# GeekAlexis/FastMOT

Measured on AMD Instinct MI355X. Metric: end-to-end tracker FPS @1080p/50 dets, higher is better.
Workload: dtype f16

## Files before the change

### fastmot_amd/_lib.py

```python
import ctypes as C
import os
import sys
import weakref
from pathlib import Path

import numpy as np
from types import SimpleNamespace

from .utils.nv12 import NV12Frame
from .utils.jpeg import JPEGFrame, QT_ENTRIES, max_coefficients
from .utils.source import SourceFrame
from .utils.yuv import PlanarFrame, frame_bytes
from .utils.packed import PackedFrame, row_bytes
from .utils.bayer import BayerFrame
from .utils.deep import DeepFrame, deep_frame_bytes
from .utils.devarray import DeviceArrayFrame

LIB_PATH = Path(os.environ.get('FASTMOT_LIB_PATH', Path(__file__).parent / 'libfastmot_hip.so'))

c_int_p = C.POINTER(C.c_int)
_lib = None


class FastMOTHipError(RuntimeError):
# ... 127 lines not shown
    check(load().fm_jpeg_encode_regions_assemble(_ptr(plans), C.c_int(len(plans)), C.c_int(int(quality)), _ptr(lens), _ptr(segs),
                                                 C.c_size_t(segs.size if segs_bytes is None else segs_bytes), _ptr(out), C.c_size_t(cap),
                                                 _ptr(offsets)))
    return [out[int(a):int(b)].tobytes() for a, b in zip(offsets[:-1], offsets[1:])]


def _redact_args(regions):
    regions = np.ascontiguousarray(regions, dtype=REDACT_REGION_DTYPE).reshape(-1)
    return regions, (_ptr(regions) if len(regions) else None, C.c_int(len(regions)))


def redact_check(regions, width, height):
    regions, args = _redact_args(regions)
    return load().fm_redact_check(*args, C.c_int(width), C.c_int(height))


def redact_render_host(frame, regions):
    if not isinstance(frame, np.ndarray) or frame.dtype != np.uint8 or frame.ndim != 3 or frame.shape[2] != 3 or \
            frame.strides[1:] != (3, 1) or frame.strides[0] < 3 * frame.shape[1] or not frame.flags.writeable:
        raise ValueError('frame must be a writeable uint8 HxWx3 array with packed pixels')
    regions, args = _redact_args(regions)
    check(load().fm_redact_render_host(_ptr(frame), C.c_int(frame.shape[1]), C.c_int(frame.shape[0]), C.c_size_t(frame.strides[0]), *args))
    return frame


def device_count():
    n = load().fm_device_count()
    if n < 0:
        raise FastMOTHipError(load().fm_last_error().decode())
    return n


def device_pci_bus_id(device):
    buf = C.create_string_buffer(64)
    check(load().fm_device_pci_bus_id(C.c_int(device), buf, C.c_int(64)))
    return buf.value.decode().lower()


class HipContext:

    def __init__(self, device=0):
        self._dev_pending = []
        self.lib = load()
        self._ctx = C.c_void_p()
        check(self.lib.fm_ctx_create(C.c_int(device), C.byref(self._ctx)))
        self.device = device
        self.feat_dim = 512

    def close(self):
        if getattr(self, '_ctx', None) is not None and self._ctx:
            self.lib.fm_ctx_destroy(self._ctx)
            self._ctx = C.c_void_p()
        for frame, _ in self._dev_pending:
            frame._pending = [(ref, t) for ref, t in frame._pending if ref() is not self]
        self._dev_pending = []

    def __del__(self):
        if sys.is_finalizing():
            return
        try:
            self.close()
        except Exception:
            pass

    @property
    def handle(self):
        return self._ctx

    def synchronize(self):
        check(self.lib.fm_ctx_synchronize(self._ctx))

    def set_option(self, key, value):
        check(self.lib.fm_ctx_set_option(self._ctx, key.encode(), C.c_int(int(value))))

    def get_option(self, key):
        v = C.c_int(0)
        check(self.lib.fm_ctx_get_option(self._ctx, key.encode(), C.byref(v)))
        return v.value

    def front_info(self):
        k, b, n = C.c_int(0), C.c_longlong(0), C.c_longlong(0)
        check(self.lib.fm_net_front_info(self._ctx, C.byref(k), C.byref(b), C.byref(n)))
        return k.value, b.value, n.value

    def trace_start(self, cap=20000):
        t0 = C.c_int64(0)
        check(self.lib.fm_trace_start(self._ctx, C.c_int(cap), C.byref(t0)))
        self._trace_cap = cap
        return t0.value

    def trace_read(self):
        cap = self._trace_cap
        tags = np.zeros(cap, np.int32)
        ms = np.zeros(cap, np.float32)
        n = C.c_int(0)
        check(self.lib.fm_trace_read(self._ctx, C.c_int(cap), _ptr(tags), _ptr(ms), C.byref(n)))
        return tags[:n.value], ms[:n.value]

    def bind_thread(self):
        check(self.lib.fm_ctx_bind_thread(self._ctx))

    def device_info(self):
        buf = C.create_string_buffer(256)
        check(self.lib.fm_device_info(self._ctx, buf, 256))
        parts = buf.value.decode().split(':')
        return {'name': parts[0], 'arch': ':'.join(parts[1:-3]), 'cus': int(parts[-3]),
                'clock_mhz': int(parts[-2]), 'hbm_bytes': int(parts[-1])}

    def kf_configure(self, dt, std_factor_acc, std_offset_acc, std_factor_det, std_factor_klt,
                     min_std_det, min_std_klt, init_pos_weight, init_vel_weight, vel_coupling,
                     vel_half_life):
        p = KFParams(dt, std_factor_acc, std_offset_acc, (C.c_double * 2)(*std_factor_det),
                     (C.c_double * 2)(*std_factor_klt), (C.c_double * 2)(*min_std_det),
                     (C.c_double * 2)(*min_std_klt), init_pos_weight, init_vel_weight, vel_coupling,
                     vel_half_life)
        check(self.lib.fm_kf_configure(self._ctx, C.byref(p)))

    def set_frame_rect(self, tlbr):
        a = _as(tlbr, np.float64, (4,))
        check(self.lib.fm_set_frame_rect(self._ctx, _ptr(a)))

    def trk_create(self, slots, det_tlbr):
        s = _as(slots, np.int32)
        b = _as(det_tlbr, np.float64, (-1, 4))
        assert len(s) == len(b)
        check(self.lib.fm_trk_create(self._ctx, C.c_int(len(s)), _ptr(s), _ptr(b)))

    def trk_step(self, slots, H, klt_tlbr, has_klt, mult):
        s = _as(slots, np.int32)
        n = len(s)
        Hm = _as(H, np.float64, (9,))
        k = _as(klt_tlbr, np.float64, (-1, 4)) if n else np.zeros((0, 4))
        hk = _as(has_klt, np.uint8)
        mu = _as(mult, np.float64)
        assert len(k) == n and len(hk) == n and len(mu) == n
        tlbr = np.empty((n, 4), np.float64)
        lost = np.empty(n, np.uint8)
        check(self.lib.fm_trk_step(self._ctx, C.c_int(n), _ptr(s), _ptr(Hm), _ptr(k), _ptr(hk),
                                   _ptr(mu), _ptr(tlbr), _ptr(lost)))
        return tlbr, lost.astype(bool)

    def trk_step_ops(self, ops, slots, H, klt_tlbr, has_klt, mult):
        s = _as(slots, np.int32)
        n = len(s)
        Hm = _as(H, np.float64, (9,))
        k = _as(klt_tlbr, np.float64, (-1, 4)) if n else np.zeros((0, 4))
        hk = _as(has_klt, np.uint8)
        mu = _as(mult, np.float64)
        tlbr = np.empty((n, 4), np.float64)
        lost = np.empty(n, np.uint8)
        check(self.lib.fm_trk_step_ops(self._ctx, C.c_int(ops), C.c_int(n), _ptr(s), _ptr(Hm), _ptr(k),
                                       _ptr(hk), _ptr(mu), _ptr(tlbr), _ptr(lost)))
        return tlbr, lost.astype(bool)

    def trk_update_det(self, slots, det_tlbr):
        s = _as(slots, np.int32)
        n = len(s)
        b = _as(det_tlbr, np.float64, (-1, 4)) if n else np.zeros((0, 4))
        assert len(b) == n
        tlbr = np.empty((n, 4), np.float64)
        lost = np.empty(n, np.uint8)
        check(self.lib.fm_trk_update_det(self._ctx, C.c_int(n), _ptr(s), _ptr(b), _ptr(tlbr), _ptr(lost)))
        return tlbr, lost.astype(bool)

    def trk_get_state(self, slots):
        s = _as(slots, np.int32)
# ... 931 lines not shown
```

### fastmot_amd/build.py

```python
import subprocess
import sys
from pathlib import Path

PKG = Path(__file__).resolve().parent
CSRC = PKG / 'csrc'
OUT = PKG / 'libfastmot_hip.so'
HIPCC = '/opt/rocm/bin/hipcc'
import os
FLAGS = ['--offload-arch=gfx950', '-O3', '-std=c++17', '-fPIC', '-shared', '-ffp-contract=off',
         '-Wno-unused-result'] + os.environ.get('FASTMOT_EXTRA_HIPCC_FLAGS', '').split()


FILE_FLAGS = {'flow.hip': ['-fno-slp-vectorize'], 'diag.hip': ['-fno-slp-vectorize'], 'reidhead_gem.hip': ['-fno-slp-vectorize']}


def sources():
    return sorted(CSRC.glob('*.hip'))


FLAGS_STAMP = PKG / 'build' / 'flags.txt'


def needs_build():
    if not OUT.exists():
        return True
    if not FLAGS_STAMP.exists() or FLAGS_STAMP.read_text() != ' '.join(FLAGS):
        return True
    t = OUT.stat().st_mtime
    deps = list(CSRC.glob('*')) + [PKG.parent / 'include' / 'fastmot_hip.h', Path(__file__)]
    return any(p.stat().st_mtime > t for p in deps)


def build(force=False, verbose=True):
    if not force and not needs_build():
        return OUT
    if FLAGS_STAMP.exists() and FLAGS_STAMP.read_text() != ' '.join(FLAGS):
        force = True
    objs = []
    procs = []
    bdir = PKG / 'build'
    bdir.mkdir(exist_ok=True)
    for src in sources():
        obj = bdir / (src.stem + '.o')
        objs.append(obj)
        if not force and obj.exists() and obj.stat().st_mtime > max(
                src.stat().st_mtime, *(h.stat().st_mtime for h in CSRC.glob('*.h')),
                (PKG.parent / 'include' / 'fastmot_hip.h').stat().st_mtime):
            continue
        cmd = [HIPCC] + [f for f in FLAGS if f != '-shared'] + FILE_FLAGS.get(src.name, []) + ['-c', str(src), '-o', str(obj)]
        procs.append((src, subprocess.Popen(cmd, stdout=subprocess.PIPE, stderr=subprocess.STDOUT)))
    for src, p in procs:
        out, _ = p.communicate()
        if p.returncode != 0:
            raise RuntimeError(f'hipcc failed on {src}:\n{out.decode()}')
        if verbose and out.strip():
            print(out.decode())
    cmd = [HIPCC, '--offload-arch=gfx950', '-shared', '-fPIC', '-o', str(OUT)] + [str(o) for o in objs]
    res = subprocess.run(cmd, stdout=subprocess.PIPE, stderr=subprocess.STDOUT)
    if res.returncode != 0:
        raise RuntimeError(f'link failed:\n{res.stdout.decode()}')
    FLAGS_STAMP.write_text(' '.join(FLAGS))
    if verbose:
        print(f'built {OUT}')
    return OUT


if __name__ == '__main__':
    build(force='--force' in sys.argv)
```

### fastmot_amd/csrc/common.h

```cpp
#pragma once
#include <hip/hip_runtime.h>
#include <atomic>
#include <cstdarg>
#include <cstdint>
#include <cstdio>
#include <cstring>
#include <string>
#include <vector>
#include "../../include/fastmot_hip.h"
#ifdef FM_DIAG
#include "../../include/fastmot_hip_diag.h"
#endif

#define FM_ERR_HIP (-1)
#define FM_ERR_ARG (-2)
#define FM_ERR_STATE (-3)

void fm_set_error(const char* fmt, ...);

#define FM_HIP(call)                                                                        \
    do {                                                                                    \
        hipError_t e_ = (call);                                                             \
        if (e_ != hipSuccess) {                                                             \
            fm_set_error("%s:%d %s -> %s", __FILE__, __LINE__, #call, hipGetErrorString(e_)); \
            return FM_ERR_HIP;                                                              \
        }                                                                                   \
    } while (0)

#define FM_CHECK_ARG(cond)                                                     \
    do {                                                                       \
        if (!(cond)) {                                                         \
            fm_set_error("%s:%d bad argument: %s", __FILE__, __LINE__, #cond); \
            return FM_ERR_ARG;                                                 \
        }                                                                      \
    } while (0)

bool fm_lap_host(const double* cost, int nr, int nc, long rs, long cs, int32_t* col4row_out);
int fm_greedy_host(const double* cost, int nr, int nc, double max_cost, int32_t* m_rows, int32_t* m_cols);
#define FM_ZERO_COPY_TRACKS (ctx->opt_zero_copy_tracks)

struct DevBuf {
    void* d = nullptr;
    void* h = nullptr;
    size_t cap = 0;
    bool pinned_mirror = true;
    int reserve(size_t bytes) {
        if (bytes <= cap) return 0;
        size_t ncap = cap ? cap : 4096;
        while (ncap < bytes) ncap *= 2;
        if (d) (void)hipFree(d);
        if (h) (void)hipHostFree(h);
        d = h = nullptr;
        cap = 0;
        FM_HIP(hipMalloc(&d, ncap));
        if (pinned_mirror) FM_HIP(hipHostMalloc(&h, ncap, hipHostMallocDefault));
        cap = ncap;
        return 0;
    }
    void release() {
        if (d) (void)hipFree(d);
        if (h) (void)hipHostFree(h);
        d = h = nullptr;
        cap = 0;
    }
    template <typename T> T* dev() { return reinterpret_cast<T*>(d); }
    template <typename T> T* host() { return reinterpret_cast<T*>(h); }
};

struct KFConst {
    double F_pos_self;
    double F_pos_other;
    double F_vel;
    double q_pp, q_pv, q_vv;
    double std_factor_acc, std_offset_acc;
    double fac_det[2], fac_klt[2], min_det[2], min_klt[2];
    double init_pos_weight, init_vel_weight;
};

struct NetState;
struct DetState;
struct ExtState;
struct FlowState;
struct EncState;
struct OvlState;
struct YuvState;
struct SsdState;
struct GalleryState;
constexpr int FM_GALLERY_CHANNELS = 2;

struct fm_ctx {
    int device = 0;
    int opt_zero_copy_tracks = 2048;
    int opt_host_lap_elems = 262144;
    int opt_use_graphs = 1;
    int opt_fused_input = 1;
    int opt_net_timing = 0;
    int opt_nms_general = 0;
    int opt_det_front_ahead = 1;
    int opt_det_front_layers = -1;
    int opt_det_front_stream = 0;
    bool det_flush_deferred = false;
    int opt_lk_variant = 0;
    void* predict_worker = nullptr;
    hipStream_t s_main = nullptr;
    hipStream_t s_det = nullptr;
    hipStream_t s_up = nullptr;
    hipStream_t s_ext = nullptr;
    hipStream_t s_ext_x[FM_MAX_EXTRA_EXTRACTORS] = {};
    hipEvent_t ev_ext_in = nullptr, ev_ext_x_done[FM_MAX_EXTRA_EXTRACTORS] = {};
    hipStream_t s_flow = nullptr;
    hipStream_t s_flow2 = nullptr;
    hipEvent_t ev_pyr = nullptr;
    bool pyr_pending = false;
    hipEvent_t ev_prep = nullptr, ev_bg = nullptr;
    hipEvent_t ev_feat = nullptr;
    hipEvent_t ev_ext_net = nullptr;
    hipEvent_t ev_ext_done = nullptr;
    hipEvent_t ev_pair = nullptr;
    bool ext_net_recorded = false;
    size_t as_in_bytes = 0;
    bool as_in_device = true;
    bool as_mirror = false;

    int slot_cap = 0;
    double* mean = nullptr;
    double* cov = nullptr;
    int feat_dim = 512;
    float* feat_sum = nullptr;
    float* feat_avg = nullptr;
    int32_t* feat_cnt = nullptr;
    KFConst kf{};
    bool kf_set = false;
    double frame_rect[4] = {0, 0, 0, 0};

    float* emb = nullptr;
    float* emb_host = nullptr;
    int emb_cap = 0;
    int emb_n = 0;

    int as_nT = 0, as_nD = 0, as_metric = 0;
    size_t as_off[6] = {0, 0, 0, 0, 0, 0};
    DevBuf as_in;
    DevBuf as_pair;
    DevBuf as_stage_in;
    DevBuf as_cost;
    DevBuf as_work;
    DevBuf as_out;
    DevBuf io0, io1;
    DevBuf occ_in, occ_out;
    DevBuf feat_in;

    int frame_w = 0, frame_h = 0, ring_size = 0;
    uint8_t* frame_cur = nullptr;
    uint8_t* frame_own = nullptr;
    uint8_t* frame_own2 = nullptr;
    uint8_t* frame_next = nullptr;
    uint8_t* frame_pinned2 = nullptr;
    hipEvent_t ev_next_upload = nullptr;
    uint8_t* frame_ahead[FM_MAX_DET_BATCH + 1] = {};
    uint8_t* frame_up[FM_MAX_DET_BATCH + 1] = {};
    uint8_t* frame_up_pinned[FM_MAX_DET_BATCH + 1] = {};
    hipEvent_t ev_up[FM_MAX_DET_BATCH + 1] = {};
    uint8_t* frame_ring = nullptr;
    uint8_t* frame_pinned = nullptr;

    DetState* det = nullptr;
    SsdState* ssd = nullptr;
    ExtState* ext = nullptr;
    NetState* det_net = nullptr;
    NetState* ext_net = nullptr;
    NetState* ext_net_x[FM_MAX_EXTRA_EXTRACTORS] = {};
    FlowState* flow = nullptr;
    EncState* enc = nullptr;
    OvlState* ovl = nullptr;
    YuvState* yuv = nullptr;
    GalleryState* gallery[2] = {nullptr, nullptr};

    std::vector<hipEvent_t> trace_ev;
// ... 123 lines not shown
```

### fastmot_amd/csrc/convd.hip

```cpp
#include "net.h"
#include <atomic>
#include <cstdlib>

int launch_convd(const ConvParams& p, hipStream_t s);

namespace {

int g_convd_cfg = 0;

#ifdef FM_CONVD_TIMING
__device__ long long g_convd_stamps[2][264];
int g_convd_abl = 0;
#define CONVD_STAMP(i) if (stamp_slot >= 0 && (i) < 264) reinterpret_cast<long long*>(smem + stamp_off)[(i)] = __builtin_readcyclecounter();
#define CONVD_ABL(bit) (abl & (bit))
#define CONVD_EXTRA_PARAM , const int abl, const int stamp_off
#define CONVD_EXTRA_ARG , g_convd_abl, (int)lds
#define CONVD_EXTRA_LDS 4096
#else
#define CONVD_STAMP(i)
#define CONVD_ABL(bit) false
#define CONVD_EXTRA_PARAM
#define CONVD_EXTRA_ARG
#define CONVD_EXTRA_LDS 0
#endif
// ... 195 lines not shown
#pragma unroll
                        for (int pi = 0; pi < MP; ++pi)
                            acc[mi][pi] = __builtin_amdgcn_mfma_f32_32x32x16_f16(af[mi], bf[pi], acc[mi][pi], 0, 0, 0);
                }
            }
            c_stage = c_stage + 1 == nslots ? 0 : c_stage + 1;
        }
        CONVD_STAMP(11 + 4 * it)
    }
    CONVD_STAMP(3)

    if constexpr (KG > 1) {
        __syncthreads();
        float4* part = reinterpret_cast<float4*>(smem + BN * LDO * 4);
        if (mfma_wave && g > 0) {
#pragma unroll
            for (int mi = 0; mi < MC; ++mi)
#pragma unroll
                for (int pi = 0; pi < MP; ++pi)
#pragma unroll
                    for (int q = 0; q < 4; ++q)
                        part[(((g - 1) * MC * MP + mi * MP + pi) * 4 + q) * 256 + w * 64 + lane] =
                            make_float4(acc[mi][pi][4 * q + 0], acc[mi][pi][4 * q + 1], acc[mi][pi][4 * q + 2], acc[mi][pi][4 * q + 3]);
        }
        __syncthreads();
        if (mfma_wave && g == 0) {
            for (int gg = 1; gg < KG; ++gg)
#pragma unroll
                for (int mi = 0; mi < MC; ++mi)
#pragma unroll
                    for (int pi = 0; pi < MP; ++pi)
#pragma unroll
                        for (int q = 0; q < 4; ++q) {
                            const float4 t4 = part[(((gg - 1) * MC * MP + mi * MP + pi) * 4 + q) * 256 + w * 64 + lane];
                            acc[mi][pi][4 * q + 0] += t4.x; acc[mi][pi][4 * q + 1] += t4.y;
                            acc[mi][pi][4 * q + 2] += t4.z; acc[mi][pi][4 * q + 3] += t4.w;
                        }
        }
    }
    CONVD_STAMP(4)
    float* so = reinterpret_cast<float*>(smem);
    if constexpr (KG == 1) __syncthreads();
    if (mfma_wave && g == 0) {
#pragma unroll
        for (int pi = 0; pi < MP; ++pi)
#pragma unroll
            for (int mi = 0; mi < MC; ++mi)
#pragma unroll
                for (int q = 0; q < 4; ++q)
                    *reinterpret_cast<float4*>(&so[((wp * MP + pi) * 32 + frow) * LDO + (wc * MC + mi) * 32 + 8 * q + 4 * fh]) =
                        make_float4(acc[mi][pi][4 * q + 0], acc[mi][pi][4 * q + 1], acc[mi][pi][4 * q + 2], acc[mi][pi][4 * q + 3]);
    }
    __syncthreads();
    constexpr int CH = BM / 8;
    constexpr int ROWS = T / CH;
    const int och = tid % CH, orow = tid / CH;
    const int co = c0 + och * 8;
    if (co < p.cout_store && !CONVD_ABL(4)) {
        const int hw_out = p.Ho * p.Wo;
        const float inv_hw = 1.f / (float)hw_out, inv_wo = 1.f / (float)p.Wo;
        float bias8[8];
        *reinterpret_cast<float4*>(&bias8[0]) = *reinterpret_cast<const float4*>(p.bias + co);
        *reinterpret_cast<float4*>(&bias8[4]) = *reinterpret_cast<const float4*>(p.bias + co + 4);
        constexpr int NPASS = (BN + ROWS - 1) / ROWS;
        float v[NPASS][8], r[NPASS][8];
#pragma unroll
        for (int ps = 0; ps < NPASS; ++ps) {
            const int row = min(orow + ps * ROWS, BN - 1);
            *reinterpret_cast<float4*>(&v[ps][0]) = *reinterpret_cast<const float4*>(&so[row * LDO + och * 8]);
            *reinterpret_cast<float4*>(&v[ps][4]) = *reinterpret_cast<const float4*>(&so[row * LDO + och * 8 + 4]);
        }
        if (p.res_mode != RES_NONE) {
#pragma unroll
            for (int ps = 0; ps < NPASS; ++ps) {
                const int pix = min(p0 + orow + ps * ROWS, p.P - 1);
                unpack8(*reinterpret_cast<const uint4*>(p.res + (size_t)pix * p.res_cs + p.res_coff + co), r[ps]);
            }
        }
#pragma unroll
        for (int ps = 0; ps < NPASS; ++ps) {
            const int row = orow + ps * ROWS;
            const int pix = p0 + row;
            if (row >= BN || pix >= p.P) continue;
#pragma unroll
            for (int e = 0; e < 8; ++e) {
                v[ps][e] += bias8[e];
                if (p.res_mode == RES_BEFORE_ACT) v[ps][e] += r[ps][e];
            }
            apply_act_n<8>(v[ps], p.act);
            if (p.res_mode == RES_AFTER_ACT) {
#pragma unroll
                for (int e = 0; e < 8; ++e) v[ps][e] += r[ps][e];
            }
            if (p.out32) {
                float* dst = p.out32 + (size_t)pix * p.out_cs + p.out_coff + co;
                *reinterpret_cast<float4*>(dst) = make_float4(v[ps][0], v[ps][1], v[ps][2], v[ps][3]);
                *reinterpret_cast<float4*>(dst + 4) = make_float4(v[ps][4], v[ps][5], v[ps][6], v[ps][7]);
            } else {
                const uint4 o = pack8(v[ps]);
                if (p.up == 2) {
                    const int nn = idiv_small(pix, hw_out, inv_hw), rem = pix - nn * hw_out;
                    const int ry = idiv_small(rem, p.Wo, inv_wo), rx = rem - ry * p.Wo;
                    const size_t o00 = ((size_t)nn * 2 * p.Ho + 2 * ry) * (2 * p.Wo) + 2 * rx;
                    f16* dst = p.out + o00 * p.out_cs + p.out_coff + co;
                    *reinterpret_cast<uint4*>(dst) = o;
                    *reinterpret_cast<uint4*>(dst + p.out_cs) = o;
                    *reinterpret_cast<uint4*>(dst + (size_t)2 * p.Wo * p.out_cs) = o;
                    *reinterpret_cast<uint4*>(dst + (size_t)(2 * p.Wo + 1) * p.out_cs) = o;
                } else {
                    *reinterpret_cast<uint4*>(p.out + (size_t)pix * p.out_cs + p.out_coff + co) = o;
                }
            }
        }
    }
    CONVD_STAMP(5)
#ifdef FM_CONVD_TIMING
    if (stamp_slot >= 0) {
        long long* st = reinterpret_cast<long long*>(smem + stamp_off);
        st[263] = __builtin_amdgcn_s_memrealtime();
        st[6] = per;
        st[7] = BM * 1000000 + BN * 1000 + KG * 100 + SPB * 10 + ns;
        for (int i = 0; i < 264; ++i) g_convd_stamps[stamp_slot][i] = st[i];
    }
#endif
#endif
}

constexpr int LDS_MAX = 160 * 1024;

struct Cfg {
    int bm, bn, kg, ns, role, spb;
};

template <int WC, int WP, int MC, int MP, int KG, int TAPS, int ROLE, int SPB>
int launch_inst(const ConvParams& p, int ns, hipStream_t s) {
    constexpr int BM = WC * MC * 32, BN = WP * MP * 32, SS = (BM + BN) * 128 * SPB;
    const int cout_pad = (p.Cout + 31) & ~31;
    const int nk = p.Kpad >> 6, per = ((nk + KG - 1) / KG + SPB - 1) / SPB;
    const int nslots = ns < per ? ns : (per < 1 ? 1 : per);
    ConvParams q = p;
    q.grid_p = (p.P + BN - 1) / BN;
    q.grid_c = (cout_pad + BM - 1) / BM;
    q.grid_z = 1;
    q.weight_major = (size_t)cout_pad * p.Kpad > (size_t)p.N * p.H * p.W * p.Cin ? 1 : 0;
    const size_t ring = (size_t)KG * nslots * SS;
    const size_t epi = (size_t)BN * (BM + 4) * 4 + (size_t)(KG - 1) * BM * BN * 4;
    const size_t lds = ring > epi ? ring : epi;
    FM_CHECK_ARG(lds + CONVD_EXTRA_LDS <= (size_t)LDS_MAX);
    static std::atomic<unsigned long long> configured{0};
    int dev = 0;
    FM_HIP(hipGetDevice(&dev));
    if (dev >= 64 || !(configured.load(std::memory_order_relaxed) >> dev & 1)) {
        FM_HIP(hipFuncSetAttribute(reinterpret_cast<const void*>(convd_kernel<WC, WP, MC, MP, KG, TAPS, ROLE, SPB>),
                                   hipFuncAttributeMaxDynamicSharedMemorySize, LDS_MAX));
        if (dev < 64) configured.fetch_or(1ull << dev, std::memory_order_relaxed);
    }
    const int total = q.grid_p * q.grid_c;
    hipLaunchKernelGGL((convd_kernel<WC, WP, MC, MP, KG, TAPS, ROLE, SPB>), dim3(((total + 7) / 8) * 8), dim3(256 * KG * (1 + ROLE)),
                       lds + CONVD_EXTRA_LDS, s, q, ns, nslots CONVD_EXTRA_ARG);
    FM_HIP(hipGetLastError());
    return 0;
}

template <int MC, int MP, int KG, int ROLE, int SPB>
int launch_taps(const ConvParams& p, int ns, hipStream_t s) {
    if (p.KH == 1) return launch_inst<2, 2, MC, MP, KG, 0, ROLE, SPB>(p, ns, s);
    return launch_inst<2, 2, MC, MP, KG, 3, ROLE, SPB>(p, ns, s);
}

template <int MC, int MP, int SPB>
int launch_role(const ConvParams& p, const Cfg& c, hipStream_t s) {
    if constexpr (MC * MP == 1 && SPB == 1) {
        if (c.kg == 4) return launch_taps<MC, MP, 4, 0, 1>(p, c.ns, s);
    }
    if (c.kg >= 2) return c.role ? launch_taps<MC, MP, 2, 1, SPB>(p, c.ns, s) : launch_taps<MC, MP, 2, 0, SPB>(p, c.ns, s);
    return c.role ? launch_taps<MC, MP, 1, 1, SPB>(p, c.ns, s) : launch_taps<MC, MP, 1, 0, SPB>(p, c.ns, s);
// ... 88 lines not shown
```

### fastmot_amd/csrc/ctx.hip

```cpp
#include <algorithm>
#include "common.h"
void convd_set_cfg(int code);
#include <sched.h>
#include <cstring>
#include <cstdlib>
#include <cmath>

static thread_local char g_err[1024] = "";

void fm_set_error(const char* fmt, ...) {
    va_list ap;
    va_start(ap, fmt);
    vsnprintf(g_err, sizeof(g_err), fmt, ap);
    va_end(ap);
}

extern "C" const char* fm_last_error(void) { return g_err; }

extern "C" int fm_ctx_set_option(fm_ctx* ctx, const char* key, int value) {
    FM_CHECK_ARG(ctx && key && (value >= 0 || (value == -1 && !strcmp(key, "det_front_layers"))));
    if (!strcmp(key, "zero_copy_tracks")) ctx->opt_zero_copy_tracks = value;
    else if (!strcmp(key, "host_lap_elems")) ctx->opt_host_lap_elems = value;
    else if (!strcmp(key, "use_graphs")) ctx->opt_use_graphs = value;
    else if (!strcmp(key, "convd_cfg")) convd_set_cfg(value);
    else if (!strcmp(key, "nms_path")) {
        ctx->opt_nms_general = value != 0;
    }
    else if (!strcmp(key, "fused_input")) ctx->opt_fused_input = value != 0;
    else if (!strcmp(key, "net_timing")) ctx->opt_net_timing = value;
    else if (!strcmp(key, "det_front_ahead") || !strcmp(key, "det_front_stream")) {
        FM_CHECK_ARG(value <= (key[10] == 'a' ? 2 : 1));
        (key[10] == 'a' ? ctx->opt_det_front_ahead : ctx->opt_det_front_stream) = value;
    }
    else if (!strcmp(key, "det_front_layers")) ctx->opt_det_front_layers = value;
    else if (!strcmp(key, "lk_variant")) {
#ifndef FM_DIAG
        if (value != 0) {
            fm_set_error("option 'lk_variant' needs a diagnostic build of the library (-DFM_DIAG)");
            return FM_ERR_ARG;
        }
#endif
        ctx->opt_lk_variant = value;
    }
    else {
        fm_set_error("unknown option '%s'", key);
        return FM_ERR_ARG;
    }
    return 0;
}

extern "C" int fm_ctx_get_option(fm_ctx* ctx, const char* key, int* value) {
    FM_CHECK_ARG(ctx && key && value);
    if (!strcmp(key, "det_front_ahead")) *value = ctx->opt_det_front_ahead;
    else if (!strcmp(key, "det_front_layers")) *value = ctx->opt_det_front_layers;
    else if (!strcmp(key, "det_front_stream")) *value = ctx->opt_det_front_stream;
    else {
        fm_set_error("option '%s' cannot be read", key);
        return FM_ERR_ARG;
    }
    return 0;
}

extern "C" int fm_trace_start(fm_ctx* ctx, int cap, int64_t* host_ns) {
    FM_CHECK_ARG(ctx && cap > 0 && host_ns && !ctx->trace_on.load() && ctx->trace_ev.empty());
    FM_HIP(hipDeviceSynchronize());
    std::vector<hipEvent_t> evs(cap);
    for (auto& e : evs) FM_HIP(hipEventCreate(&e));
    if (!ctx->trace_base) FM_HIP(hipEventCreate(&ctx->trace_base));
    FM_HIP(hipEventRecord(ctx->trace_base, ctx->s_main));
    FM_HIP(hipEventSynchronize(ctx->trace_base));
    timespec ts;
    clock_gettime(CLOCK_MONOTONIC, &ts);
    *host_ns = (int64_t)ts.tv_sec * 1000000000ll + ts.tv_nsec;
    ctx->trace_tag.assign(cap, 0);
    ctx->trace_n = 0;
    ctx->trace_ev = std::move(evs);
    ctx->trace_on.store(true, std::memory_order_release);
    return 0;
}

extern "C" int fm_trace_read(fm_ctx* ctx, int cap, int32_t* tags, float* ms, int* n) {
    FM_CHECK_ARG(ctx && tags && ms && n);
    ctx->trace_on.store(false, std::memory_order_seq_cst);
    while (ctx->trace_busy.load(std::memory_order_seq_cst) > 0) sched_yield();
    FM_HIP(hipDeviceSynchronize());
    std::vector<hipEvent_t> evs = std::move(ctx->trace_ev);
    ctx->trace_ev.clear();
    int k = ctx->trace_n.load();
    if (k > (int)evs.size()) k = (int)evs.size();
    if (k > cap) k = cap;
    for (int i = 0; i < k; ++i) {
        tags[i] = ctx->trace_tag[i];
        FM_HIP(hipEventElapsedTime(&ms[i], ctx->trace_base, evs[i]));
    }
    *n = k;
    for (auto& e : evs) (void)hipEventDestroy(e);
    return 0;
}

extern "C" int fm_ctx_bind_thread(fm_ctx* ctx) {
    FM_CHECK_ARG(ctx);
    FM_HIP(hipSetDevice(ctx->device));
    return 0;
}

extern "C" int fm_device_pci_bus_id(int device, char* buf, int buflen) {
    FM_CHECK_ARG(buf && buflen >= 16);
    FM_HIP(hipDeviceGetPCIBusId(buf, buflen, device));
    return 0;
}

extern "C" int fm_device_count(void) {
    int n = 0;
    FM_HIP(hipGetDeviceCount(&n));
    return n;
}

void fm_net_free(NetState* n);
void fm_det_free(DetState* d);
void fm_ext_free(ExtState* e);
void fm_flow_free(FlowState* f);

extern "C" int fm_ctx_create(int device, fm_ctx** out) {
    FM_CHECK_ARG(out != nullptr);
    int n = 0;
    FM_HIP(hipGetDeviceCount(&n));
    if (device < 0 || device >= n) {
        fm_set_error("device %d out of range (%d visible)", device, n);
        return FM_ERR_ARG;
    }
    FM_HIP(hipSetDevice(device));
    fm_ctx* ctx = new fm_ctx();
    ctx->device = device;
    if (const char* e = getenv("FASTMOT_ZERO_COPY")) ctx->opt_zero_copy_tracks = atoi(e);
    if (const char* e = getenv("FASTMOT_HOST_LAP")) ctx->opt_host_lap_elems = atoi(e);
    if (const char* e = getenv("FASTMOT_GRAPHS")) ctx->opt_use_graphs = atoi(e);
    if (const char* e = getenv("FASTMOT_FUSED_INPUT")) ctx->opt_fused_input = atoi(e) != 0;
    if (const char* e = getenv("FASTMOT_FRONT_AHEAD")) ctx->opt_det_front_ahead = std::min(std::max(atoi(e), 0), 2);
    if (const char* e = getenv("FASTMOT_FRONT_STREAM")) ctx->opt_det_front_stream = atoi(e) == 1;
    int prio_lo = 0, prio_hi = 0;
    FM_HIP(hipDeviceGetStreamPriorityRange(&prio_lo, &prio_hi));
    const int prio_det = prio_lo, prio_ext = prio_hi;
    FM_HIP(hipStreamCreateWithPriority(&ctx->s_main, hipStreamNonBlocking, prio_hi));
    FM_HIP(hipStreamCreateWithPriority(&ctx->s_det, hipStreamNonBlocking, prio_det));
    FM_HIP(hipStreamCreateWithPriority(&ctx->s_up, hipStreamNonBlocking, prio_lo));
    FM_HIP(hipStreamCreateWithPriority(&ctx->s_ext, hipStreamNonBlocking, prio_ext));
    FM_HIP(hipEventCreateWithFlags(&ctx->ev_ext_in, hipEventDisableTiming));
    for (int i = 0; i < FM_MAX_EXTRA_EXTRACTORS; ++i) {
        FM_HIP(hipStreamCreateWithPriority(&ctx->s_ext_x[i], hipStreamNonBlocking, prio_hi));
        FM_HIP(hipEventCreateWithFlags(&ctx->ev_ext_x_done[i], hipEventDisableTiming));
    }
    FM_HIP(hipStreamCreateWithPriority(&ctx->s_flow, hipStreamNonBlocking, prio_hi));
    FM_HIP(hipStreamCreateWithPriority(&ctx->s_flow2, hipStreamNonBlocking, prio_hi));
    FM_HIP(hipEventCreateWithFlags(&ctx->ev_pyr, hipEventDisableTiming));
    FM_HIP(hipEventCreateWithFlags(&ctx->ev_prep, hipEventDisableTiming));
    FM_HIP(hipEventCreateWithFlags(&ctx->ev_bg, hipEventDisableTiming));
    FM_HIP(hipEventCreateWithFlags(&ctx->ev_feat, hipEventDisableTiming));
    FM_HIP(hipEventCreateWithFlags(&ctx->ev_ext_net, hipEventDisableTiming));
    FM_HIP(hipEventCreateWithFlags(&ctx->ev_pair, hipEventDisableTiming));
    FM_HIP(hipEventCreateWithFlags(&ctx->ev_ext_done, hipEventDisableTiming));
    int rc = fm_ensure_slots(ctx, 1024);
    if (rc) return rc;
    *out = ctx;
    return 0;
}

extern "C" int fm_ctx_destroy(fm_ctx* ctx) {
    if (!ctx) return 0;
    (void)hipSetDevice(ctx->device);
    fm_predict_worker_free(ctx);
    fm_gallery_free(ctx);
    (void)hipDeviceSynchronize();
    if (ctx->det) fm_det_free(ctx->det);
    fm_ssd_free(ctx);
    if (ctx->ext) fm_ext_free(ctx->ext);
    for (void* p : {(void*)ctx->frame_own, (void*)ctx->frame_own2, (void*)ctx->frame_ring})
        if (p) (void)hipFree(p);
    if (ctx->frame_pinned) (void)hipHostFree(ctx->frame_pinned);
    if (ctx->frame_pinned2) (void)hipHostFree(ctx->frame_pinned2);
    for (int k = 2; k <= FM_MAX_DET_BATCH; ++k) {
        if (ctx->frame_up[k]) (void)hipFree(ctx->frame_up[k]);
        if (ctx->frame_up_pinned[k]) (void)hipHostFree(ctx->frame_up_pinned[k]);
        if (ctx->ev_up[k]) (void)hipEventDestroy(ctx->ev_up[k]);
    }
    for (hipEvent_t e : ctx->ev_jpeg)
        if (e) (void)hipEventDestroy(e);
    fm_frame_dev_free(ctx);
    fm_frame_staging_free(ctx);
    fm_overlay_free(ctx);
    fm_yuv_free(ctx);
    fm_jpegenc_free(ctx);
    if (ctx->det_net) fm_net_free(ctx->det_net);
    if (ctx->ext_net) fm_net_free(ctx->ext_net);
    for (NetState* x : ctx->ext_net_x)
        if (x) fm_net_free(x);
    if (ctx->flow) fm_flow_free(ctx->flow);
    for (void* p : {(void*)ctx->mean, (void*)ctx->cov, (void*)ctx->feat_sum, (void*)ctx->feat_avg,
                    (void*)ctx->feat_cnt, (void*)ctx->emb})
        if (p) (void)hipFree(p);
    if (ctx->emb_host) (void)hipHostFree(ctx->emb_host);
    for (DevBuf* b : {&ctx->as_in, &ctx->as_pair, &ctx->as_stage_in, &ctx->as_cost, &ctx->as_work,
                      &ctx->as_out, &ctx->io0, &ctx->io1, &ctx->feat_in, &ctx->occ_in, &ctx->occ_out})
        b->release();
    for (hipStream_t s : {ctx->s_main, ctx->s_det, ctx->s_up, ctx->s_ext, ctx->s_flow, ctx->s_flow2})
        if (s) (void)hipStreamDestroy(s);
    for (hipEvent_t e : {ctx->ev_feat, ctx->ev_ext_in, ctx->ev_pyr, ctx->ev_prep, ctx->ev_bg, ctx->ev_ext_net, ctx->ev_pair, ctx->ev_ext_done})
        if (e) (void)hipEventDestroy(e);
    for (int i = 0; i < FM_MAX_EXTRA_EXTRACTORS; ++i) {
        if (ctx->s_ext_x[i]) (void)hipStreamDestroy(ctx->s_ext_x[i]);
        if (ctx->ev_ext_x_done[i]) (void)hipEventDestroy(ctx->ev_ext_x_done[i]);
    }
    delete ctx;
    return 0;
}

extern "C" int fm_ctx_synchronize(fm_ctx* ctx) {
    FM_CHECK_ARG(ctx);
    FM_HIP(hipStreamSynchronize(ctx->s_main));
    FM_HIP(hipStreamSynchronize(ctx->s_det));
    FM_HIP(hipStreamSynchronize(ctx->s_up));
// ... 345 lines not shown
```

### fastmot_amd/csrc/detect.hip

```cpp
#include "pixel_source.h"
#include <cmath>
#include <string>
#include <vector>

struct DetState {
    fm_yolo_cfg cfg{};
    bool configured = false;
    int cap = 8192;
    static constexpr int NSLOT_UNTILED = FM_MAX_DET_BATCH + 2;
    static constexpr int NSLOT = 3 * FM_MAX_DET_BATCH;
    int nslot = NSLOT_UNTILED;
    int n_tiles = 0;
    int tile_x[FM_MAX_DET_BATCH] = {}, tile_y[FM_MAX_DET_BATCH] = {};
    int region_w = 0, region_h = 0;
    double tile_offset[FM_MAX_DET_BATCH][2] = {};
    double merge_thresh = 0.6;
    std::vector<fm_det48> tile_stage;
    std::vector<fm_det48> tile_dets;
    std::vector<int32_t> tile_ids;
    int tile_count[FM_MAX_DET_BATCH] = {};
    int tile_sum[2] = {};
    float* cand[NSLOT] = {};
    float* sorted[NSLOT] = {};
    int32_t* counters[NSLOT] = {};
// ... 606 lines not shown
}

static int detect_ahead(fm_ctx* ctx, int n) {
    FM_CHECK_ARG(ctx && ctx->det_net && n >= 1 && n <= FM_MAX_DET_BATCH);
    if (n > ctx->det_net->max_batch) {
        fm_set_error("detector look-ahead of %d frames > the detector network's max_batch %d", n, ctx->det_net->max_batch);
        return FM_ERR_ARG;
    }
    const uint8_t* frames[FM_MAX_DET_BATCH];
    hipEvent_t uploads[FM_MAX_DET_BATCH];
    for (int k = 1; k <= n; ++k) {
        frames[k - 1] = fm_ahead_frame(ctx, k);
        if (!frames[k - 1]) {
            fm_set_error("look-ahead slot %d holds no frame (fm_frame_upload_ahead / fm_frame_ring_select_ahead)", k);
            return FM_ERR_ARG;
        }
        uploads[k - 1] = frames[k - 1] == fm_ahead_buf(ctx, k) ? fm_ahead_event(ctx, k) : nullptr;
    }
    return detect_pass(ctx, frames, uploads, n, true);
}

static int detect_pass(fm_ctx* ctx, const uint8_t* const* frames, const hipEvent_t* uploads, int n, bool look_ahead) {
    FM_CHECK_ARG(ctx && ctx->det && ctx->det->configured && ctx->det_net);
    DetState* d = ctx->det;
    NetState* net = ctx->det_net;
    const fm_yolo_cfg& c = d->cfg;
    const bool tiled = d->n_tiles > 1;
    const int n_frames = n;
    if (tiled) {
        FM_CHECK_ARG(n_frames == 1);
        n = d->n_tiles;
        if (n > net->max_batch) {
            fm_set_error("%d tiles > the detector network's max_batch %d", n, net->max_batch);
            return FM_ERR_ARG;
        }
    }
    FM_CHECK_ARG(n >= 1 && n <= FM_MAX_DET_BATCH && n <= net->max_batch);
    hipStream_t s = ctx->s_det;
    int rc = 0;
    const bool fused = ctx->opt_fused_input && fm_net_stem_fusable(net, c.input_tensor);
    int K = 0;
    if (ctx->det_flush_deferred && !(look_ahead && fused && n == 1 && !tiled)) {
        ctx->det_flush_deferred = false;
        if ((rc = flush_post(ctx, d))) return rc;
    }
    if (look_ahead && fused && n == 1 && !tiled && ctx->opt_det_front_ahead && ctx->opt_det_front_layers) {
        bool busy = ctx->opt_det_front_ahead == 2;
        if (!busy && d->pending > 0 && hipEventQuery(d->ev_dec[(d->wr + d->nslot - 1) % d->nslot]) != hipSuccess) {
            (void)hipGetLastError();
            busy = true;
        }
        if (busy && (rc = fm_net_front_prepare(ctx, net, ctx->opt_det_front_layers, &K))) return rc;
    }
    if (ctx->det_flush_deferred && !K) {
        ctx->det_flush_deferred = false;
        if ((rc = flush_post(ctx, d))) return rc;
    }
    const bool timing = ctx->opt_net_timing > 0 && d->n_passes++ % ctx->opt_net_timing == 0;
    for (int i = 0; i < n; ++i) {
        d->timed[(d->wr + i) % d->nslot] = timing && i == 0;
        d->timed_front[(d->wr + i) % d->nslot] = timing && i == 0 && K > 0;
    }
    struct Restore {
        NetState* net;
        ~Restore() { net->first = net->last = 0; fm_net_select(net, nullptr, net->set); }
    } restore{net};
    fm_trace_mark(ctx, s, 10);
    if (K > 0) {
        hipStream_t se = ctx->opt_det_front_stream == 1 ? ctx->s_ext : ctx->s_up;
        const int set = net->set ^ 1;
        if (net->front_stream && net->front_stream != se) FM_HIP(hipStreamSynchronize(net->front_stream));
        net->front_stream = se;
        ++net->front_passes;
        if (uploads[0] && se != ctx->s_ext) FM_HIP(hipStreamWaitEvent(se, uploads[0], 0));
        if ((rc = acquire_slots(ctx, d, se, 1))) return rc;
        if (d->set_slot[set] >= 0 && hipEventQuery(d->ev_dec[d->set_slot[set]]) != hipSuccess) {
            (void)hipGetLastError();
            FM_HIP(hipStreamWaitEvent(se, d->ev_dec[d->set_slot[set]], 0));
        }
        const StemSrc src = det_source(ctx, d, frames, n);
        fm_net_select(net, se, set);
        if (timing) FM_HIP(hipEventRecord(d->evf0[d->wr], se));
        fm_trace_mark(ctx, se, 11);
        if ((rc = fm_net_run_stem_from(ctx, net, src, n))) return rc;
        fm_trace_mark(ctx, se, 15);
        if (K > 1) {
            net->first = 1;
            net->last = K;
            if ((rc = fm_net_run_internal(ctx, FM_NET_DETECTOR, n))) return rc;
        }
        if (timing) FM_HIP(hipEventRecord(d->evf1[d->wr], se));
        fm_trace_mark(ctx, se, 16);
        FM_HIP(hipEventRecord(d->ev_front[set], se));
        if (ctx->det_flush_deferred) {
            ctx->det_flush_deferred = false;
            if ((rc = flush_post(ctx, d))) return rc;
        }
        fm_net_select(net, nullptr, set);
        FM_HIP(hipStreamWaitEvent(s, d->ev_front[set], 0));
        fm_trace_mark(ctx, s, 14);
        if (timing) FM_HIP(hipEventRecord(d->ev0[d->wr], s));
        net->first = K;
        net->last = 0;
        if ((rc = fm_net_run_internal(ctx, FM_NET_DETECTOR, n))) return rc;
        net->first = 0;
    } else {
        for (int i = 0; i < n_frames; ++i)
            if (uploads[i]) FM_HIP(hipStreamWaitEvent(s, uploads[i], 0));
        if ((rc = acquire_slots(ctx, d, s, n))) return rc;
        fm_trace_mark(ctx, s, 14);
        const StemSrc src = det_source(ctx, d, frames, n);
        if (fused) {
            if (timing) FM_HIP(hipEventRecord(d->ev0[d->wr], s));
            fm_trace_mark(ctx, s, 11);
            if ((rc = fm_net_run_stem_from(ctx, net, src, n))) return rc;
            fm_trace_mark(ctx, s, 15);
            net->first = 1;
            rc = fm_net_run_internal(ctx, FM_NET_DETECTOR, n);
            net->first = 0;
            if (rc) return rc;
        } else {
            if ((rc = enqueue_preprocess(ctx, d, net, src, n))) return rc;
            if (timing) FM_HIP(hipEventRecord(d->ev0[d->wr], s));
            fm_trace_mark(ctx, s, 11);
            if ((rc = fm_net_run_internal(ctx, FM_NET_DETECTOR, n))) return rc;
        }
    }
    d->set_slot[net->set] = d->wr;
    if (timing) FM_HIP(hipEventRecord(d->ev1[d->wr], s));
    fm_trace_mark(ctx, s, 12);
    FilterArgs fa = filter_args(d, d->wr);
    HeadSet hs{};
    for (int i = 0; i < n; ++i) {
        const int slot = (d->wr + i) % d->nslot;
        hs.cand[i] = d->cand[slot];
        hs.counters[i] = d->counters[slot];
    }
    for (int i = 0; i < FM_MAX_DET_BATCH; ++i) {
        hs.off_x[i] = tiled && i < n ? d->tile_offset[i][0] : c.offset[0];
        hs.off_y[i] = tiled && i < n ? d->tile_offset[i][1] : c.offset[1];
    }
    int base = 0, blocks = 0;
    for (int i = 0; i < FM_MAX_HEADS + 1; ++i) hs.first_block[i] = 0x7fffffff;
    for (int i = 0; i < c.n_heads; ++i) {
        FM_CHECK_ARG(c.head_tensor[i] >= 0 && c.head_tensor[i] < (int)net->tensors.size());
        const fm_tensor& t = net->tensors[c.head_tensor[i]];
        FM_CHECK_ARG(t.f32 && t.h == c.grid_h[i] && t.w == c.grid_w[i] && c.n_anchors[i] <= FM_MAX_ANCHORS);
        HeadArgs& h = hs.h[i];
        h.data = (const float*)net->bufs[c.head_tensor[i]];
        h.cs = t.c; h.gw = c.grid_w[i]; h.gh = c.grid_h[i]; h.na = c.n_anchors[i];
        h.base_index = base;
        memcpy(h.anchors, c.anchors[i], sizeof(float) * 2 * FM_MAX_ANCHORS);
        h.scale_xy = c.scale_xy[i];
        const int cnt = h.gw * h.gh * h.na;
        hs.first_block[i] = blocks;
        blocks += (cnt + 255) / 256;
        base += cnt;
    }
    if (blocks) hipLaunchKernelGGL(decode_kernel, dim3(blocks, n), dim3(256), 0, s, hs, fa, c.in_w, c.in_h, c.new_coords);
    FM_HIP(hipGetLastError());
    fm_trace_mark(ctx, s, 13);
    return enqueue_post(ctx, d, s, n);
}

extern "C" int fm_detect_sync(fm_ctx* ctx, fm_det48* out, int cap, int* n) {
    FM_CHECK_ARG(ctx && ctx->det && ctx->det->configured && out && n);
    if (ctx->det->n_tiles > 1) return collect_tiles(ctx, ctx->det, ctx->s_det, out, cap, n);
    return collect(ctx, ctx->det, ctx->s_det, out, cap, n);
}

extern "C" int fm_filter_dets(fm_ctx* ctx, const float* rows, int n, fm_det48* out, int cap, int* n_out) {
    FM_CHECK_ARG(ctx && ctx->det && ctx->det->configured && n >= 0 && out && n_out);
    FM_CHECK_ARG(n < (1 << FM_SORT_INDEX_BITS));
    DetState* d = ctx->det;
    hipStream_t s = ctx->s_det;
    FM_HIP(hipStreamSynchronize(s));
    FM_HIP(hipStreamSynchronize(ctx->s_up));
    if (int rc_n = fm_net_sync(ctx->det_net)) return rc_n;
    d->set_slot[0] = d->set_slot[1] = -1;
    d->post_pending = -1;
    d->post_pending_n = 0;
    d->rd = d->wr;
    d->pending = 0;
    if (n > d->rows_cap) {
        if (d->rows_in) FM_HIP(hipFree(d->rows_in));
        d->rows_in = nullptr;
        FM_HIP(hipMalloc(&d->rows_in, sizeof(float) * 7 * (size_t)n));
        d->rows_cap = n;
    }
    if (n) FM_HIP(hipMemcpyAsync(d->rows_in, rows, sizeof(float) * 7 * (size_t)n, hipMemcpyHostToDevice, s));
    FM_HIP(hipMemsetAsync(d->counters[d->wr], 0, sizeof(int32_t) * 4, s));
    if (n) hipLaunchKernelGGL(rows_filter_kernel, dim3((n + 255) / 256), dim3(256), 0, s, d->rows_in, n, filter_args(d, d->wr));
    int rc = enqueue_post(ctx, d, s);
    if (rc) return rc;
    return collect(ctx, d, s, out, cap, n_out);
}

extern "C" int fm_detect_last_counts(fm_ctx* ctx, int* n_candidates, int* n_detections) {
    FM_CHECK_ARG(ctx && ctx->det && n_candidates && n_detections);
    const DetState* d = ctx->det;
// ... 56 lines not shown
```

### fastmot_amd/csrc/extract.hip

```cpp
#include "pixel_source.h"
#include <cmath>

struct ExtState {
    int input_tensor = -1, in_w = 0, in_h = 0;
    double* boxes = nullptr;
    double* boxes_host = nullptr;
    int cap = 0;
    DevBuf emb_out;
    int exported_n = -1;
    bool mirror_export = false;
};

void fm_ext_invalidate_export(fm_ctx* ctx) {
    if (ctx->ext) ctx->ext->exported_n = -1;
}

void fm_ext_free(ExtState* e) {
    if (!e) return;
    e->emb_out.release();
    if (e->boxes) (void)hipFree(e->boxes);
    if (e->boxes_host) (void)hipHostFree(e->boxes_host);
    delete e;
}

namespace {

__global__ __launch_bounds__(256) void export_kernel(const float4* __restrict__ src, float4* __restrict__ dst, int n4) {
    for (int i = blockIdx.x * 256 + threadIdx.x; i < n4; i += gridDim.x * 256) dst[i] = src[i];
}

__global__ void crop_resize_kernel(const uint8_t* __restrict__ frame, int fw, int fh,
                                   const double* __restrict__ boxes, int n, f16* __restrict__ out,
                                   int ow, int oh, int cs) {
    const int x = blockIdx.x * blockDim.x + threadIdx.x;
    const int y = blockIdx.y, b = blockIdx.z;
    if (x >= ow) return;
    f16x8 o;
    crop_input_pixel(frame, fw, fh, boxes + (size_t)b * 4, x, y, ow, oh, o);
    *reinterpret_cast<f16x8*>(out + (((size_t)b * oh + y) * ow + x) * cs) = o;
}

}

extern "C" int fm_extract_configure(fm_ctx* ctx, int input_tensor, int in_w, int in_h) {
    FM_CHECK_ARG(ctx && ctx->ext_net && input_tensor >= 0 && input_tensor < (int)ctx->ext_net->tensors.size());
    const fm_tensor& t = ctx->ext_net->tensors[input_tensor];
    FM_CHECK_ARG(t.h == in_h && t.w == in_w && !t.f32);
    if (!ctx->ext) ctx->ext = new ExtState();
    ctx->ext->input_tensor = input_tensor;
    ctx->ext->in_w = in_w;
    ctx->ext->in_h = in_h;
    return 0;
}

int fm_emb_reserve(fm_ctx* ctx, int n);
bool fm_net_writes_mirror(const NetState* net);

static int export_embeddings(fm_ctx* ctx, ExtState* e, int n, hipStream_t s) {
    const size_t bytes = sizeof(float) * (size_t)n * ctx->feat_dim;
    e->exported_n = -1;
    if (ctx->emb_host && fm_net_writes_mirror(ctx->ext_net)) {
        e->exported_n = n;
        e->mirror_export = true;
        FM_HIP(hipEventRecord(ctx->ev_ext_done, s));
        return 0;
    }
    e->mirror_export = false;
    if (bytes > e->emb_out.cap) {
        FM_HIP(hipStreamSynchronize(s));
        int rc = e->emb_out.reserve(bytes);
        if (rc) return rc;
    }
    const int n4 = (int)(bytes / 16);
    hipLaunchKernelGGL(export_kernel, dim3((n4 + 255) / 256 < 64 ? (n4 + 255) / 256 : 64), dim3(256), 0, s,
                       (const float4*)ctx->emb, (float4*)e->emb_out.h, n4);
    FM_HIP(hipGetLastError());
    e->exported_n = n;
    FM_HIP(hipEventRecord(ctx->ev_ext_done, s));
    return 0;
}

static int front_end(fm_ctx* ctx, ExtState* e, NetState* ni, hipStream_t si, int off, int b, int cs) {
    ni->first = 0;
    if (ctx->opt_fused_input && fm_net_stem_fusable(ni, e->input_tensor)) {
        StemSrc src{};
        src.kind = 2; src.frame[0] = ctx->frame_cur; src.fw = ctx->frame_w; src.fh = ctx->frame_h;
        src.boxes = e->boxes_host + (size_t)off * 4;
        int rc = fm_net_run_stem_from(ctx, ni, src, b);
        if (rc) return rc;
        ni->first = 1;
        return 0;
    }
    hipLaunchKernelGGL(crop_resize_kernel, dim3((e->in_w + 127) / 128, e->in_h, b), dim3(128), 0, si,
                       ctx->frame_cur, ctx->frame_w, ctx->frame_h, e->boxes + (size_t)off * 4, b,
                       (f16*)ni->bufs[e->input_tensor], e->in_w, e->in_h, cs);
    FM_HIP(hipGetLastError());
    return 0;
}

extern "C" int fm_extract_async(fm_ctx* ctx, int n, const double* tlbr) {
    FM_CHECK_ARG(ctx && ctx->ext && ctx->ext_net && n >= 0 && ctx->frame_cur);
    ctx->emb_n = 0;
    ctx->ext_net_recorded = false;
    int rc_exp = 0;
    if (ctx->ext) ctx->ext->exported_n = -1;
    if (n == 0) return 0;
    FM_CHECK_ARG(tlbr);
    ExtState* e = ctx->ext;
    NetState* net = ctx->ext_net;
    hipStream_t s = ctx->s_ext;
    if (n > e->cap) {
        FM_HIP(hipStreamSynchronize(s));
        if (e->boxes) FM_HIP(hipFree(e->boxes));
        if (e->boxes_host) FM_HIP(hipHostFree(e->boxes_host));
        e->boxes = e->boxes_host = nullptr;
        int cap = e->cap ? e->cap : 64;
        while (cap < n) cap *= 2;
        FM_HIP(hipMalloc(&e->boxes, sizeof(double) * 4 * cap));
        FM_HIP(hipHostMalloc(&e->boxes_host, sizeof(double) * 4 * cap, hipHostMallocDefault));
        e->cap = cap;
    }
    if (hipEventQuery(ctx->ev_feat) != hipSuccess) {
        (void)hipGetLastError();
        FM_HIP(hipStreamWaitEvent(s, ctx->ev_feat, 0));
    }
    if (n > ctx->emb_cap) {
        FM_HIP(hipStreamSynchronize(ctx->s_main));
        FM_HIP(hipStreamSynchronize(s));
        int rc = fm_emb_reserve(ctx, n);
        if (rc) return rc;
    }
    FM_HIP(hipStreamSynchronize(s));
    memcpy(e->boxes_host, tlbr, sizeof(double) * 4 * n);
    const bool zero_copy_boxes = ctx->opt_fused_input && fm_net_stem_fusable(net, e->input_tensor);
    if (!zero_copy_boxes)
        FM_HIP(hipMemcpyAsync(e->boxes, e->boxes_host, sizeof(double) * 4 * n, hipMemcpyHostToDevice, s));
    fm_trace_mark(ctx, s, 32);
    const fm_tensor& t = net->tensors[e->input_tensor];
    int parts = 1;
    while (parts <= FM_MAX_EXTRA_EXTRACTORS && ctx->ext_net_x[parts - 1]) ++parts;
    while (parts > 1 && n < 4 * parts) --parts;
    if (parts > 1 && (n + parts - 1) / parts <= net->max_batch) {
        FM_HIP(hipEventRecord(ctx->ev_ext_in, s));
        int off = 0;
        for (int i = 0; i < parts; ++i) {
            const int b = n / parts + (i < n % parts ? 1 : 0);
            NetState* ni = i == 0 ? net : ctx->ext_net_x[i - 1];
            hipStream_t si = i == 0 ? s : ctx->s_ext_x[i - 1];
            FM_CHECK_ARG(b <= ni->max_batch);
            if (i) FM_HIP(hipStreamWaitEvent(si, ctx->ev_ext_in, 0));
            int rc = front_end(ctx, e, ni, si, off, b, t.c);
            if (rc) return rc;
            ni->emb_offset = off;
            rc = fm_net_run_internal(ctx, i == 0 ? FM_NET_EXTRACTOR : FM_NET_EXTRACTOR_B + i - 1, b);
            ni->emb_offset = 0;
            ni->first = 0;
            if (rc) return rc;
            if (i) {
                FM_HIP(hipEventRecord(ctx->ev_ext_x_done[i - 1], si));
                FM_HIP(hipStreamWaitEvent(s, ctx->ev_ext_x_done[i - 1], 0));
            }
            off += b;
        }
        FM_HIP(hipEventRecord(ctx->ev_ext_net, s));
        ctx->ext_net_recorded = true;
        if ((rc_exp = export_embeddings(ctx, e, n, s))) return rc_exp;
        fm_trace_mark(ctx, s, 33);
        ctx->emb_n = n;
        return 0;
    }
    for (int off = 0; off < n; off += net->max_batch) {
        const int b = n - off < net->max_batch ? n - off : net->max_batch;
        int rc = front_end(ctx, e, net, s, off, b, t.c);
// ... 61 lines not shown
```

### fastmot_amd/csrc/net.h

```cpp
#pragma once
#include "common.h"
#include <hip/hip_fp16.h>

typedef _Float16 f16;
typedef f16 f16x8 __attribute__((ext_vector_type(8)));
typedef f16 f16x4 __attribute__((ext_vector_type(4)));
typedef float f32x16 __attribute__((ext_vector_type(16)));
typedef float f32x4 __attribute__((ext_vector_type(4)));

enum { ACT_LINEAR = 0, ACT_LEAKY = 1, ACT_MISH = 2, ACT_RELU = 3, ACT_LOGISTIC = 4, ACT_SWISH = 5, ACT_RELU6 = 6 };
enum { RES_NONE = 0, RES_AFTER_ACT = 1, RES_BEFORE_ACT = 2 };

struct ConvParams {
    const f16* in;  int in_cs, in_coff;
    const f16* w;
    const float* bias;
    f16* out;       int out_cs, out_coff;
    float* out32;
    const f16* res; int res_cs, res_coff;
    int N, H, W, Cin, Ho, Wo, Cout, KH, KW, stride, pad;
    int K, Kpad, P;
    int cout_store;
    int act, res_mode;
    int grid_p, grid_c, grid_z, weight_major;
    int pad_dx;
    int up;
    int batch_inv;
};

int launch_conv(const ConvParams& p, float* ws, size_t ws_floats, hipStream_t s);

struct NetState {
    int which = 0, max_batch = 0;
    std::vector<fm_tensor> tensors;
    std::vector<void*> bufs;
    std::vector<fm_layer> layers;
    char* weights = nullptr;
    size_t weight_bytes = 0;
    float* gates = nullptr;
    int n_gates = 0, gate_c = 0;
    hipStream_t stream = nullptr;
    char* arena = nullptr;
    float* ws = nullptr;
    size_t ws_floats = 0;
    struct GraphKey {
        long batch_emb;
        int first, last, set;
        bool operator==(const GraphKey& o) const { return batch_emb == o.batch_emb && first == o.first && last == o.last && set == o.set; }
    };
    std::vector<std::pair<GraphKey, hipGraphExec_t>> graphs;
    bool use_graphs = true;
    int emb_offset = 0;
    int batch_offset = 0;
    int first = 0;
    int last = 0;
    int front_k = 0;
    int front_req = 0;
    int set = 0;
    std::vector<void*> bufs_b;
    std::vector<char> in_front;
    std::vector<void*> front_owned;
    float* ws_b = nullptr;
    size_t front_bytes = 0;
    hipStream_t home = nullptr;
    hipStream_t front_stream = nullptr;
    long front_passes = 0;
};

int fm_net_front_prepare(fm_ctx* ctx, NetState* net, int request, int* k);
void fm_net_select(NetState* net, hipStream_t s, int set);
int fm_net_sync(NetState* net);

NetState* fm_net_get(fm_ctx* ctx, int which);
int fm_net_run_internal(fm_ctx* ctx, int which, int batch);

__device__ __forceinline__ void unpack8(const uint4& v, float* f) {
    const f16x8 h = *reinterpret_cast<const f16x8*>(&v);
#pragma unroll
    for (int e = 0; e < 8; ++e) f[e] = (float)h[e];
}
__device__ __forceinline__ uint4 pack8(const float* f) {
    f16x8 h;
#pragma unroll
    for (int e = 0; e < 8; ++e) h[e] = (f16)f[e];
    return *reinterpret_cast<const uint4*>(&h);
}

__device__ __forceinline__ int idiv_small(int i, int d, float inv) {
    (void)d;
    return (int)(((float)i + 0.5f) * inv);
}

template <int HI>
__device__ __forceinline__ float fma_mix_h(uint32_t packed, float k, float acc) {
    float d;
    if constexpr (HI) asm("v_fma_mix_f32 %0, %1, %2, %3 op_sel:[1,0,0] op_sel_hi:[1,0,0]" : "=v"(d) : "v"(packed), "v"(k), "v"(acc));
    else asm("v_fma_mix_f32 %0, %1, %2, %3 op_sel:[0,0,0] op_sel_hi:[1,0,0]" : "=v"(d) : "v"(packed), "v"(k), "v"(acc));
    return d;
}
template <int HI>
__device__ __forceinline__ float fma_mix_hh(uint32_t packed, uint32_t kpacked, float acc) {
    float d;
    if constexpr (HI) asm("v_fma_mix_f32 %0, %1, %2, %3 op_sel:[1,1,0] op_sel_hi:[1,1,0]" : "=v"(d) : "v"(packed), "v"(kpacked), "v"(acc));
    else asm("v_fma_mix_f32 %0, %1, %2, %3 op_sel:[0,0,0] op_sel_hi:[1,1,0]" : "=v"(d) : "v"(packed), "v"(kpacked), "v"(acc));
    return d;
}
template <int N>
__device__ __forceinline__ void fma_mix_nh(const uint32_t* raw, const uint32_t* k, float* acc) {
#pragma unroll
    for (int e = 0; e < N; e += 2) {
        acc[e] = fma_mix_hh<0>(raw[e >> 1], k[e >> 1], acc[e]);
        acc[e + 1] = fma_mix_hh<1>(raw[e >> 1], k[e >> 1], acc[e + 1]);
    }
}
template <int N>
__device__ __forceinline__ void fma_mix_n(const uint32_t* raw, const float* k, float* acc) {
#pragma unroll
    for (int e = 0; e < N; e += 2) {
        acc[e] = fma_mix_h<0>(raw[e >> 1], k[e], acc[e]);
        acc[e + 1] = fma_mix_h<1>(raw[e >> 1], k[e + 1], acc[e + 1]);
    }
}

__device__ __forceinline__ void store_out(const ConvParams& p, long pix, int co, f16x4 o) {
    if (p.up == 2) {
        const int hw = p.Ho * p.Wo, rem = (int)(pix % hw);
        const size_t o00 = ((size_t)(pix / hw) * 2 * p.Ho + 2 * (rem / p.Wo)) * (2 * p.Wo) + 2 * (rem % p.Wo);
        f16* dst = p.out + o00 * p.out_cs + p.out_coff + co;
        *reinterpret_cast<f16x4*>(dst) = o;
        *reinterpret_cast<f16x4*>(dst + p.out_cs) = o;
        *reinterpret_cast<f16x4*>(dst + (size_t)2 * p.Wo * p.out_cs) = o;
        *reinterpret_cast<f16x4*>(dst + (size_t)(2 * p.Wo + 1) * p.out_cs) = o;
    } else {
        *reinterpret_cast<f16x4*>(p.out + (size_t)pix * p.out_cs + p.out_coff + co) = o;
    }
}

__device__ __forceinline__ float act_rcp(float x) { return __builtin_amdgcn_rcpf(x); }
__device__ __forceinline__ float act_leaky(float x) { return x > 0.f ? x : 0.1f * x; }
__device__ __forceinline__ float act_relu(float x) { return x > 0.f ? x : 0.f; }
__device__ __forceinline__ float act_relu6(float x) { return fminf(fmaxf(x, 0.f), 6.f); }
__device__ __forceinline__ float act_mish(float x) {
    const float n = __expf(x);
    const float t = n * (n + 2.f);
    return x > 20.f ? x : x * (t * act_rcp(t + 2.f));
}
__device__ __forceinline__ float act_logistic(float x) { return act_rcp(1.f + __expf(-x)); }
__device__ __forceinline__ float act_swish(float x) { return x * act_rcp(1.f + __expf(-x)); }

__device__ __forceinline__ float apply_act(float x, int act) {
    switch (act) {
        case ACT_LEAKY: return act_leaky(x);
        case ACT_MISH: return act_mish(x);
        case ACT_RELU: return act_relu(x);
        case ACT_LOGISTIC: return act_logistic(x);
        case ACT_SWISH: return act_swish(x);
        case ACT_RELU6: return act_relu6(x);
        default: return x;
    }
}

template <int N>
__device__ __forceinline__ void apply_act_n(float* v, int act) {
    switch (act) {
        case ACT_LEAKY:
#pragma unroll
            for (int e = 0; e < N; ++e) v[e] = act_leaky(v[e]);
            break;
        case ACT_MISH:
#pragma unroll
            for (int e = 0; e < N; ++e) v[e] = act_mish(v[e]);
            break;
        case ACT_RELU:
#pragma unroll
            for (int e = 0; e < N; ++e) v[e] = act_relu(v[e]);
            break;
        case ACT_LOGISTIC:
#pragma unroll
            for (int e = 0; e < N; ++e) v[e] = act_logistic(v[e]);
            break;
        case ACT_SWISH:
#pragma unroll
            for (int e = 0; e < N; ++e) v[e] = act_swish(v[e]);
            break;
        case ACT_RELU6:
#pragma unroll
            for (int e = 0; e < N; ++e) v[e] = act_relu6(v[e]);
            break;
        default: break;
    }
}
```

### fastmot_amd/csrc/net.hip

```cpp
#include "pixel_source.h"
#include <algorithm>
#include <memory>

int launch_dwconv3(const f16* in, int in_cs, int in_coff, f16* out, int out_cs, int out_coff, const f16* w,
                   const float* bias, int N, int H, int W, int C, int act, hipStream_t s);
int launch_dwconv(const f16* in, int in_cs, int in_coff, f16* out, int out_cs, int out_coff, const f16* w,
                  const float* bias, int N, int H, int W, int Ho, int Wo, int C, int stride, int act, hipStream_t s);
bool sepconv_supported(int cin, int cout, int stride);
int launch_sepconv(const f16* in, int in_cs, int in_coff, f16* out, int out_cs, int out_coff, const f16* wdw,
                   const float* bdw, const f16* wpw, const float* bpw, int N, int H, int W, int Ho, int Wo, int cin,
                   int cout, int stride, int act1, int act2, long p_choice, hipStream_t s);
int launch_liteconv(int G, const f16* const* in, const int* in_cs, const int* in_coff, f16* out, int out_cs,
                    int out_coff, const f16* wpw, int kpad, const f16* wdw, const float* bias, int N, int H,
                    int W, int C, int act, float* gap_out, hipStream_t s);
void liteconv_tiling(int C, int W, int H, int* th, int* tw, int* tiles_x, int* tiles_y);
int launch_litechain(const f16* in, int in_cs, int in_coff, f16* out, int out_cs, int out_coff, const f16* wpw,
                     int kpad, const f16* wdw, const float* bias, int N, int H, int W, int C, int act,
                     float* const* gap, hipStream_t s);
int launch_gated_sum(int nstreams, const f16* const* in, const int* in_cs, const int* in_coff, int N, int HW,
                     int C, int hid, const f16* w1, const float* b1, const f16* w2, const float* b2, f16* out,
                     int out_cs, int out_coff, const float* const* part, int tiles, hipStream_t s);
constexpr int GATE_SLOT_TILES = 32;
int launch_pair11(const f16* xa, int xa_cs, int xa_coff, const f16* xc, int xc_cs, int xc_coff, f16* out, int out_cs,
                  int out_coff, const f16* w1, const float* b1, const f16* w2, const float* b2, long P, int cout, int act1,
                  int act2, hipStream_t s, long p_choice);
bool pair11_supported(int cin, int mid, int extra, int cout);
int launch_ostail(const f16* in, int in_cs, int in_coff, const f16* ph, const float* pf, int N, float* out, float* raw_out,
                  float* mirror, hipStream_t s);
bool ostail_supported(int in_h, int in_w, int cin, int mid, int cout, int feat, int n_halfs, int n_floats);
int launch_stemconv(const f16* in, int in_cs, int in_coff, f16* out, int out_cs, int out_coff, const f16* w,
                    const float* bias, int N, int H, int W, int Ho, int Wo, int k, int stride, int pad, int cout,
                    int act, hipStream_t s);
int launch_spp(const f16* in, int in_cs, int in_coff, f16* out, int out_cs, int out_coff, int N, int H, int W,
               int C, hipStream_t s);
int launch_pool(const f16* in, int in_cs, int in_coff, f16* out, int out_cs, int out_coff, int N, int H,
                int W, int C, int Ho, int Wo, int k, int stride, int pad, int avg, hipStream_t s);
int launch_upsample2(const f16* in, int in_cs, int in_coff, f16* out, int out_cs, int out_coff, int N, int H,
                     int W, int C, hipStream_t s);
int launch_conv_streamed(const ConvParams& p, hipStream_t s);
int launch_convd(const ConvParams& p, hipStream_t s);
bool resblock_supported(int C, int M);
int launch_resblock(const f16* x, int x_cs, int x_coff, f16* out, int out_cs, int out_coff, const f16* w1,
                    const float* b1, const f16* w2, const float* b2, int N, int H, int W, int C, int M, int act1,
                    int act2, hipStream_t s);
int launch_add(const f16* a, int a_cs, int a_coff, const f16* b, int b_cs, int b_coff, f16* out, int out_cs,
               int out_coff, long npix, int C, hipStream_t s);
int launch_copy(const f16* in, int in_cs, int in_coff, f16* out, int out_cs, int out_coff, long npix, int C,
                hipStream_t s);
int launch_gate(const f16* in, int in_cs, int in_coff, int N, int HW, int C, int hid, const f16* w1,
                const float* b1, const f16* w2, const float* b2, float* gate, hipStream_t s);
int launch_gate_sum(int nstreams, const f16* const* in, const int* in_cs, const int* in_coff,
                    const float* const* gate, f16* out, int out_cs, int out_coff, int N, int HW, int C,
                    hipStream_t s);
int launch_head(const f16* in, int in_cs, int in_coff, int N, int HW, int C, int D, const f16* w,
                const float* b, float* out, float* raw_out, hipStream_t s, float* mirror = nullptr);
int launch_poolhead(const f16* in, int in_cs, int in_coff, int N, int HW, int C, int D, const float* scale, const float* shift,
                    const f16* w, const float* b, int relu, float* out, float* mirror, hipStream_t s, float gem_p, float gem_eps);
int launch_instnorm(const f16* in, int in_cs, int in_coff, f16* out, int out_cs, int out_coff, int N, int HW, int C, int cn,
                    const float* gamma, const float* beta, float eps, int act, hipStream_t s, const f16* res = nullptr, int res_cs = 0,
                    int res_coff = 0);
bool convin_supported(int K, int cout, int hw);
int launch_convin(const f16* in, int in_cs, int in_coff, f16* out, int out_cs, int out_coff, const f16* res, int res_cs, int res_coff,
                  int res_mode, const f16* w, const float* bias, const float* gamma, const float* beta, int N, int HW, int K,
                  int cout, float eps, int act, hipStream_t s);
bool nonlocal_supported(int C, int hw);
int launch_nonlocal(const f16* in, int in_cs, int in_coff, f16* out, int out_cs, int out_coff, int N, int HW, int C, const float* w3,
                    const float* bias3, const float* wa, const float* wb, hipStream_t s);
int fm_emb_reserve(fm_ctx* ctx, int n);


void fm_net_free(NetState* n) {
    if (!n) return;
    for (size_t i = 0; i < n->bufs.size(); ++i)
        if (n->bufs[i] && n->tensors[i].offset < 0 && !(i < n->in_front.size() && n->in_front[i])) (void)hipFree(n->bufs[i]);
    for (void* p : n->front_owned) (void)hipFree(p);
    if (n->arena) (void)hipFree(n->arena);
    if (n->weights) (void)hipFree(n->weights);
    if (n->gates) (void)hipFree(n->gates);
    if (n->ws) (void)hipFree(n->ws);
    if (n->ws_b) (void)hipFree(n->ws_b);
    for (auto& g : n->graphs) (void)hipGraphExecDestroy(g.second);
    delete n;
}

int fm_net_sync(NetState* net) {
    if (!net) return 0;
    if (net->front_stream) FM_HIP(hipStreamSynchronize(net->front_stream));
    FM_HIP(hipStreamSynchronize(net->home ? net->home : net->stream));
    return 0;
}

void fm_net_select(NetState* net, hipStream_t s, int set) {
    net->stream = s ? s : net->home;
    if (set != net->set && !net->bufs_b.empty()) {
        net->bufs.swap(net->bufs_b);
        net->set = set;
    }
}

static NetState*& net_slot(fm_ctx* ctx, int which) {
    return which == FM_NET_DETECTOR ? ctx->det_net : which == FM_NET_EXTRACTOR ? ctx->ext_net
                                                    : ctx->ext_net_x[which - FM_NET_EXTRACTOR_B];
}
extern "C" int fm_net_front_info(fm_ctx* ctx, int* k, long long* bytes, long long* passes) {
    FM_CHECK_ARG(ctx && k && bytes && passes);
    const NetState* net = ctx->det_net;
    *k = net ? net->front_k : 0;
    *bytes = net ? (long long)net->front_bytes : 0;
    *passes = net ? (long long)net->front_passes : 0;
    return 0;
}
NetState* fm_net_get(fm_ctx* ctx, int which) { return net_slot(ctx, which); }
int fm_net_run_internal(fm_ctx* ctx, int which, int batch) { return fm_net_run(ctx, which, batch); }

void fm_net_drop_graphs(NetState* net) {
    if (!net) return;
    (void)fm_net_sync(net);
    for (auto& g : net->graphs) (void)hipGraphExecDestroy(g.second);
    net->graphs.clear();
}

static size_t elem_size(const fm_tensor& t);

constexpr size_t FRONT_BUDGET = (size_t)512 << 20;
constexpr size_t FRONT_WS_FLOATS = (size_t)16 << 20;
int fm_net_front_prepare(fm_ctx* ctx, NetState* net, int request, int* k) {
    FM_CHECK_ARG(ctx && net && k && request != 0);
    if (net->front_req == request) { *k = net->front_k; return 0; }
    const int nl = (int)net->layers.size(), nt = (int)net->tensors.size();
    const int input = net->layers[0].in[0];
    int K = 0;
    if (request > 0) K = std::min(request, nl - 1);
    else
        while (K < nl - 1 && (long)net->tensors[net->layers[K].out].h * net->tensors[net->layers[K].out].w >= 8192) ++K;
    auto plain = [](int op) {
        switch (op) {
            case FM_OP_CONV: case FM_OP_CONVS: case FM_OP_CONVD: case FM_OP_DWCONV3: case FM_OP_DWCONV: case FM_OP_SEPCONV:
            case FM_OP_STEMCONV: case FM_OP_STEM2: case FM_OP_STEMPOOL: case FM_OP_PAIR11: case FM_OP_SPP: case FM_OP_MAXPOOL:
            case FM_OP_AVGPOOL: case FM_OP_UPSAMPLE2: case FM_OP_RESBLOCK: case FM_OP_ADD: case FM_OP_COPY: case FM_OP_INSTNORM: case FM_OP_CONVIN:
            case FM_OP_NONLOCAL: return true;
            default: return false;
        }
    };
    std::vector<char> want;
    size_t bytes = 0;
    for (;; --K) {
        want.assign(nt, 0);
        bytes = net->ws_b ? 0 : FRONT_WS_FLOATS * sizeof(float);
        bool ok = true;
        for (int i = 0; i < K && ok; ++i) {
            const fm_layer& L = net->layers[i];
            ok = plain(L.op);
            want[L.out] = 1;
            for (int j = 0; j < L.n_in; ++j) want[L.in[j]] = 1;
            if (L.res_mode != FM_RES_NONE) want[L.res] = 1;
        }
        want[input] = 0;
        for (int t = 0; t < nt; ++t)
            if (want[t] && !(t < (int)net->in_front.size() && net->in_front[t])) {
                const fm_tensor& T = net->tensors[t];
                bytes += 2 * (((size_t)net->max_batch * T.h * T.w * T.c * elem_size(T) + 255) & ~(size_t)255);
            }
        if (K == 0 || (ok && net->front_bytes + bytes <= FRONT_BUDGET)) break;
    }
    net->front_req = request;
    net->front_k = K;
    *k = K;
    if (K == 0) return 0;
    fm_net_drop_graphs(net);
    if (net->in_front.empty()) {
        net->in_front.assign(nt, 0);
        net->bufs_b = net->bufs;
    }
    if (!net->ws_b) {
        FM_HIP(hipMalloc(&net->ws_b, FRONT_WS_FLOATS * sizeof(float)));
        net->front_bytes += FRONT_WS_FLOATS * sizeof(float);
    }
    for (int t = 0; t < nt; ++t) {
        if (!want[t] || net->in_front[t]) continue;
        const fm_tensor& T = net->tensors[t];
        const size_t b = (size_t)net->max_batch * T.h * T.w * T.c * elem_size(T);
        void* two[2] = {nullptr, nullptr};
        for (void*& p : two) {
            FM_HIP(hipMalloc(&p, b));
            net->front_owned.push_back(p);
            FM_HIP(hipMemset(p, 0, b));
        }
        if (T.offset < 0) FM_HIP(hipFree(net->bufs[t]));
        net->bufs[t] = two[0];
        net->bufs_b[t] = two[1];
        net->in_front[t] = 1;
        net->front_bytes += 2 * ((b + 255) & ~(size_t)255);
    }
    FM_HIP(hipStreamSynchronize(nullptr));
    return 0;
}

static size_t elem_size(const fm_tensor& t) { return t.f32 ? 4 : 2; }

extern "C" int fm_net_destroy(fm_ctx* ctx, int which) {
    FM_CHECK_ARG(ctx && (which >= 0 && which < FM_NET_EXTRACTOR_B + FM_MAX_EXTRA_EXTRACTORS));
    NetState*& slot = net_slot(ctx, which);
    if (slot) {
        int rc = fm_net_sync(slot);
        if (rc) return rc;
        fm_net_free(slot);
        slot = nullptr;
    }
    return 0;
}

extern "C" int fm_net_create(fm_ctx* ctx, int which, int max_batch, int n_tensors, const fm_tensor* tensors,
                             int n_layers, const fm_layer* layers, const void* weights, size_t weight_bytes,
                             int n_gates, int gate_channels, size_t arena_bytes) {
    FM_CHECK_ARG(ctx && (which >= 0 && which < FM_NET_EXTRACTOR_B + FM_MAX_EXTRA_EXTRACTORS) && max_batch > 0 && n_tensors > 0 && n_layers > 0);
    FM_CHECK_ARG(tensors && layers && weights && weight_bytes > 0);
    int rc = fm_net_destroy(ctx, which);
    if (rc) return rc;
    std::unique_ptr<NetState, void (*)(NetState*)> net(new NetState(), fm_net_free);
    net->which = which;
    net->max_batch = max_batch;
    net->stream = which == FM_NET_DETECTOR ? ctx->s_det : which == FM_NET_EXTRACTOR ? ctx->s_ext
                                                        : ctx->s_ext_x[which - FM_NET_EXTRACTOR_B];
    net->home = net->stream;
    net->tensors.assign(tensors, tensors + n_tensors);
    net->layers.assign(layers, layers + n_layers);
    if (arena_bytes) {
        FM_HIP(hipMalloc(&net->arena, arena_bytes));
        FM_HIP(hipMemset(net->arena, 0, arena_bytes));
    }
    for (const fm_tensor& t : net->tensors) {
        FM_CHECK_ARG(t.h > 0 && t.w > 0 && t.c > 0 && t.c % 8 == 0);
        void* b = nullptr;
        const size_t bytes = (size_t)max_batch * t.h * t.w * t.c * elem_size(t);
        if (t.offset >= 0) {
            FM_CHECK_ARG(t.offset % 256 == 0 && (size_t)t.offset + bytes <= arena_bytes);
            b = net->arena + t.offset;
        } else {
            FM_HIP(hipMalloc(&b, bytes));
            FM_HIP(hipMemset(b, 0, bytes));
        }
        net->bufs.push_back(b);
    }
    for (const fm_layer& L : net->layers) {
        FM_CHECK_ARG(L.out >= 0 && L.out < n_tensors && L.n_in >= 1 && L.n_in <= 4);
        for (int i = 0; i < L.n_in; ++i) FM_CHECK_ARG(L.in[i] >= 0 && L.in[i] < n_tensors);
        FM_CHECK_ARG(L.res_mode == FM_RES_NONE || (L.res >= 0 && L.res < n_tensors));
        FM_CHECK_ARG(L.w_off >= 0 && (size_t)L.w_off <= weight_bytes && L.w_off % 16 == 0 && L.b_off % 16 == 0);
        if (L.op == FM_OP_OSTAIL)
            FM_CHECK_ARG(L.stride > 0 && L.pad > 0 && L.b_off >= 0 && (size_t)L.w_off + (size_t)L.stride * 2 <= weight_bytes &&
                         (size_t)L.b_off + (size_t)L.pad * 4 <= weight_bytes);
    }
    FM_HIP(hipMalloc(&net->weights, weight_bytes));
    FM_HIP(hipMemcpy(net->weights, weights, weight_bytes, hipMemcpyHostToDevice));
    net->weight_bytes = weight_bytes;
    net->n_gates = n_gates;
    net->gate_c = gate_channels;
    net->ws_floats = ((size_t)16 << 20) * (which == FM_NET_DETECTOR ? (size_t)std::min(max_batch, FM_MAX_DET_BATCH) : 1);
    FM_HIP(hipMalloc(&net->ws, net->ws_floats * sizeof(float)));
    if (n_gates > 0) {
        FM_CHECK_ARG(gate_channels > 0);
        FM_HIP(hipMalloc(&net->gates, sizeof(float) * (size_t)n_gates * max_batch * gate_channels * GATE_SLOT_TILES));
    }
    if (which != FM_NET_DETECTOR) {
        FM_HIP(hipStreamSynchronize(ctx->s_main));
        if ((rc = fm_emb_reserve(ctx, max_batch))) return rc;
    }
    net_slot(ctx, which) = net.release();
    return 0;
}

static int run_layer(fm_ctx* ctx, NetState* net, const fm_layer& L, int B) {
    const fm_tensor& ti = net->tensors[L.in[0]];
    const fm_tensor& to = net->tensors[L.out];
    hipStream_t s = net->stream;
    const bool away = s != net->home && net->ws_b;
    float* ws = away ? net->ws_b : net->ws;
    const size_t ws_floats = away ? FRONT_WS_FLOATS : net->ws_floats;
    const f16* in0 = (const f16*)net->bufs[L.in[0]];
    f16* out = (f16*)net->bufs[L.out];
    switch (L.op) {
        case FM_OP_CONV:
        case FM_OP_CONVS:
        case FM_OP_CONVD: {
            ConvParams p{};
            p.in = in0; p.in_cs = ti.c; p.in_coff = L.in_coff[0];
            p.w = (const f16*)(net->weights + L.w_off);
            p.bias = (const float*)(net->weights + L.b_off);
            p.out = to.f32 ? nullptr : out;
            p.out32 = to.f32 ? (float*)net->bufs[L.out] : nullptr;
            p.out_cs = to.c; p.out_coff = L.out_coff;
            if (L.res_mode != FM_RES_NONE) {
                p.res = (const f16*)net->bufs[L.res];
                p.res_cs = net->tensors[L.res].c;
                p.res_coff = L.res_coff;
            }
            p.up = L.up == 2 ? 2 : 1;
            FM_CHECK_ARG(L.up <= 2 && (p.up == 1 || (!to.f32 && to.h % 2 == 0 && to.w % 2 == 0)));
            p.N = B; p.H = ti.h; p.W = ti.w; p.Cin = L.cin; p.Ho = to.h / p.up; p.Wo = to.w / p.up; p.Cout = L.cout;
            p.KH = p.KW = L.k; p.stride = L.stride; p.pad = L.pad;
            p.K = L.k * L.k * L.cin; p.Kpad = (p.K + 63) & ~63; p.P = B * p.Ho * p.Wo;
            p.cout_store = (L.cout + 7) & ~7;
            p.act = L.act; p.res_mode = L.res_mode;
            p.batch_inv = net->which == FM_NET_DETECTOR ? 1 : 0;
            {
                const int pad_x = L.gate[0] >= 0 && L.op != FM_OP_CONVD ? L.gate[0] : L.pad;
                const bool same2 = L.k == 3 && L.stride == 2 && L.op != FM_OP_CONVD;
                FM_CHECK_ARG(pad_x <= L.k / 2 && (pad_x == L.pad || same2));
                FM_CHECK_ARG((ti.h + 2 * L.pad - L.k) / L.stride + 1 == p.Ho || (same2 && L.pad == 0 && ti.h % 2 == 0 && p.Ho == ti.h / 2));
                FM_CHECK_ARG((ti.w + 2 * pad_x - L.k) / L.stride + 1 == p.Wo || (same2 && pad_x == 0 && ti.w % 2 == 0 && p.Wo == ti.w / 2));
                p.pad_dx = pad_x - L.pad;
            }
            FM_CHECK_ARG(L.out_coff + p.cout_store <= to.c && L.in_coff[0] + L.cin <= ti.c);
            if (L.op == FM_OP_CONVS) return launch_conv_streamed(p, s);
            if (L.op == FM_OP_CONVD) return launch_convd(p, s);
            return launch_conv(p, ws, ws_floats, s);
        }
        case FM_OP_DWCONV3:
            return launch_dwconv3(in0, ti.c, L.in_coff[0], out, to.c, L.out_coff,
                                  (const f16*)(net->weights + L.w_off), (const float*)(net->weights + L.b_off),
                                  B, ti.h, ti.w, L.cin, L.act, s);
        case FM_OP_DWCONV:
            FM_CHECK_ARG(!to.f32 && L.k == 3 && L.in_coff[0] + L.cin <= ti.c && L.out_coff + L.cin <= to.c);
            return launch_dwconv(in0, ti.c, L.in_coff[0], out, to.c, L.out_coff, (const f16*)(net->weights + L.w_off),
                                 (const float*)(net->weights + L.b_off), B, ti.h, ti.w, to.h, to.w, L.cin, L.stride, L.act, s);
        case FM_OP_SEPCONV:
            FM_CHECK_ARG(!to.f32 && L.k == 3 && sepconv_supported(L.cin, L.cout, L.stride) && L.in_coff[0] + L.cin <= ti.c &&
                         L.out_coff + L.cout <= to.c && L.gate[0] >= 0);
            FM_CHECK_ARG(L.w2_off >= 0 && L.w2_off % 16 == 0 && L.b2_off >= 0 && L.b2_off % 16 == 0 &&
                         (size_t)L.w_off + (size_t)9 * L.cin * 2 <= net->weight_bytes && (size_t)L.b_off + (size_t)L.cin * 4 <= net->weight_bytes &&
                         (size_t)L.w2_off + (size_t)((L.cout + 31) / 32) * ((L.cin + 15) / 16) * 1024 <= net->weight_bytes &&
                         (size_t)L.b2_off + (size_t)((L.cout + 31) / 32) * 128 <= net->weight_bytes);
            return launch_sepconv(in0, ti.c, L.in_coff[0], out, to.c, L.out_coff, (const f16*)(net->weights + L.w_off),
                                  (const float*)(net->weights + L.b_off), (const f16*)(net->weights + L.w2_off),
                                  (const float*)(net->weights + L.b2_off), B, ti.h, ti.w, to.h, to.w, L.cin, L.cout, L.stride,
                                  L.gate[0], L.act, net->which == FM_NET_DETECTOR ? (long)to.h * to.w : (long)B * to.h * to.w, s);
        case FM_OP_LITECONV: {
            FM_CHECK_ARG(L.cin == ((L.cout + 7) & ~7) && L.n_in >= 1 && L.n_in <= 4);
            FM_CHECK_ARG(L.out_coff + L.n_in * L.cin <= to.c);
            const f16* ins[4];
// ... 151 lines not shown
                         (size_t)L.w_off + (size_t)L.hid * 4 <= wb && (size_t)L.b_off + (size_t)L.hid * 4 <= wb);
            FM_CHECK_ARG((L.act == FM_ACT_LINEAR || L.act == FM_ACT_RELU) && eps >= 0.f && eps < 1.f);
            const f16* res = nullptr;
            int res_cs = 0;
            if (L.res_mode != FM_RES_NONE) {
                const fm_tensor& tr = net->tensors[L.res];
                FM_CHECK_ARG(L.res_mode == FM_RES_BEFORE_ACT && L.res != L.out && !tr.f32 && tr.h == ti.h && tr.w == ti.w &&
                             L.res_coff >= 0 && L.res_coff % 8 == 0 && L.res_coff + L.cin <= tr.c);
                res = (const f16*)net->bufs[L.res];
                res_cs = tr.c;
            }
            return launch_instnorm(in0, ti.c, L.in_coff[0], out, to.c, L.out_coff, B, ti.h * ti.w, L.cin, L.hid,
                                   (const float*)(net->weights + L.w_off), (const float*)(net->weights + L.b_off), eps, L.act, s,
                                   res, res_cs, L.res_coff);
        }
        case FM_OP_CONVIN: {
            const size_t wb = net->weight_bytes;
            const size_t cp = (size_t)((L.cout + 31) / 32) * 32;
            float eps;
            memcpy(&eps, &L.gate[0], sizeof eps);
            FM_CHECK_ARG(!ti.f32 && !to.f32 && L.out != L.in[0] && to.h == ti.h && to.w == ti.w && L.k == 1 && L.stride == 1 &&
                         L.pad == 0 && convin_supported(L.cin, L.cout, ti.h * ti.w));
            FM_CHECK_ARG(L.in_coff[0] >= 0 && L.out_coff >= 0 && L.in_coff[0] % 8 == 0 && L.out_coff % 8 == 0 &&
                         L.in_coff[0] + L.cin <= ti.c && L.out_coff + L.cout <= to.c);
            FM_CHECK_ARG(L.w_off >= 0 && L.b_off >= 0 && L.w2_off >= 0 && L.b2_off >= 0 && L.w2_off % 16 == 0 && L.b2_off % 16 == 0 &&
                         (size_t)L.w_off + cp * (size_t)((L.cin + 15) / 16) * 32 <= wb && (size_t)L.b_off + cp * 4 <= wb &&
                         (size_t)L.w2_off + cp * 4 <= wb && (size_t)L.b2_off + cp * 4 <= wb);
            FM_CHECK_ARG((L.act == FM_ACT_LINEAR || L.act == FM_ACT_RELU) && eps >= 0.f && eps < 1.f);
            const f16* res = nullptr;
            int res_cs = 0;
            if (L.res_mode != FM_RES_NONE) {
                const fm_tensor& tr = net->tensors[L.res];
                FM_CHECK_ARG((L.res_mode == FM_RES_BEFORE_ACT || L.res_mode == FM_RES_BEFORE_NORM) && L.res != L.out && !tr.f32 &&
                             tr.h == ti.h && tr.w == ti.w && L.res_coff >= 0 && L.res_coff % 8 == 0 && L.res_coff + L.cout <= tr.c);
                res = (const f16*)net->bufs[L.res];
                res_cs = tr.c;
            }
            return launch_convin(in0, ti.c, L.in_coff[0], out, to.c, L.out_coff, res, res_cs, L.res_coff, L.res_mode,
                                 (const f16*)(net->weights + L.w_off), (const float*)(net->weights + L.b_off),
                                 (const float*)(net->weights + L.w2_off), (const float*)(net->weights + L.b2_off), B, ti.h * ti.w,
                                 L.cin, L.cout, eps, L.act, s);
        }
        case FM_OP_NONLOCAL: {
            const size_t wb = net->weight_bytes, cb = (size_t)L.cin * 4;
            FM_CHECK_ARG(!ti.f32 && !to.f32 && L.out != L.in[0] && to.h == ti.h && to.w == ti.w && L.cout == L.cin &&
                         nonlocal_supported(L.cin, ti.h * ti.w) && L.res_mode == FM_RES_NONE && L.act == FM_ACT_LINEAR);
            FM_CHECK_ARG(L.in_coff[0] >= 0 && L.out_coff >= 0 && L.in_coff[0] % 8 == 0 && L.out_coff % 8 == 0 &&
                         L.in_coff[0] + L.cin <= ti.c && L.out_coff + L.cin <= to.c);
            FM_CHECK_ARG(L.w_off >= 0 && L.b_off >= 0 && L.w2_off >= 0 && L.b2_off >= 0 && L.w_off % 16 == 0 && L.b_off % 16 == 0 &&
                         L.w2_off % 16 == 0 && L.b2_off % 16 == 0 && (size_t)L.w_off + 3 * cb <= wb && (size_t)L.b_off + 16 <= wb &&
                         (size_t)L.w2_off + cb <= wb && (size_t)L.b2_off + cb <= wb);
            return launch_nonlocal(in0, ti.c, L.in_coff[0], out, to.c, L.out_coff, B, ti.h * ti.w, L.cin,
                                   (const float*)(net->weights + L.w_off), (const float*)(net->weights + L.b_off),
                                   (const float*)(net->weights + L.w2_off), (const float*)(net->weights + L.b2_off), s);
        }
        case FM_OP_POOLHEAD: {
            const bool neck = L.gate[0] > 0, fc = L.gate[1] > 0;
            const size_t wb = net->weight_bytes;
            float gem_p = 0.f, gem_eps = 0.f;
            if (L.gate[2] > 0) {
                memcpy(&gem_p, &L.gate[2], sizeof gem_p);
                memcpy(&gem_eps, &L.gate[3], sizeof gem_eps);
                FM_CHECK_ARG(gem_p >= 0.5f && gem_p <= 16.f && gem_eps > 0.f && gem_eps <= 1.f);
            }
            FM_CHECK_ARG(L.cout == ctx->feat_dim && net->emb_offset + B <= ctx->emb_cap && !ti.f32 && L.cin > 0 && L.cout > 0 &&
                         L.in_coff[0] + L.cin <= ti.c && (fc || L.cout == L.cin));
            FM_CHECK_ARG(!fc || (L.b_off >= 0 && (size_t)L.w_off + (size_t)L.cout * L.cin * 2 <= wb && (size_t)L.b_off + (size_t)L.cout * 4 <= wb));
            FM_CHECK_ARG(!neck || (L.w2_off >= 0 && L.b2_off >= 0 && L.w2_off % 16 == 0 && L.b2_off % 16 == 0 &&
                                   (size_t)L.w2_off + (size_t)L.cin * 4 <= wb && (size_t)L.b2_off + (size_t)L.cin * 4 <= wb));
            return launch_poolhead(in0, ti.c, L.in_coff[0], B, ti.h * ti.w, L.cin, L.cout,
                                   neck ? (const float*)(net->weights + L.w2_off) : nullptr,
                                   neck ? (const float*)(net->weights + L.b2_off) : nullptr,
                                   fc ? (const f16*)(net->weights + L.w_off) : nullptr,
                                   fc ? (const float*)(net->weights + L.b_off) : nullptr, L.act == FM_ACT_RELU,
                                   ctx->emb + (size_t)net->emb_offset * ctx->feat_dim,
                                   ctx->emb_host ? ctx->emb_host + (size_t)net->emb_offset * ctx->feat_dim : nullptr, s, gem_p, gem_eps);
        }
        default:
            fm_set_error("unknown layer op %d", L.op);
            return FM_ERR_ARG;
    }
}

bool fm_net_writes_mirror(const NetState* net) {
    if (!net || net->layers.empty()) return false;
    const int op = net->layers.back().op;
    return op == FM_OP_HEAD || op == FM_OP_OSTAIL || op == FM_OP_POOLHEAD;
}

static int run_layers_eager(fm_ctx* ctx, NetState* net, int batch) {
    const size_t end = net->last > 0 ? (size_t)net->last : net->layers.size();
    for (size_t i = (size_t)net->first; i < end; ++i) {
        int rc = run_layer(ctx, net, net->layers[i], batch);
        if (rc) return rc;
    }
    return 0;
}

bool fm_net_stem_fusable(const NetState* net, int input_tensor) {
    if (!net || net->layers.empty()) return false;
    const fm_layer& L = net->layers[0];
    if ((L.op != FM_OP_STEMCONV && L.op != FM_OP_STEM2 && L.op != FM_OP_STEMPOOL) || L.n_in != 1 || L.in[0] != input_tensor || L.in_coff[0] != 0) return false;
    for (size_t i = 1; i < net->layers.size(); ++i) {
        const fm_layer& M = net->layers[i];
        for (int k = 0; k < M.n_in; ++k)
            if (M.in[k] == input_tensor) return false;
        if (M.res_mode != FM_RES_NONE && M.res == input_tensor) return false;
        if (M.out == input_tensor) return false;
    }
    return true;
}

int launch_stem2_layer(const fm_layer& L, const StemSrc& src, const NetState* net, int batch, hipStream_t s) {
    const fm_tensor& ti = net->tensors[L.in[0]];
    const fm_tensor& to = net->tensors[L.out];
    const bool three = L.gate[1] > 0;
    const int cout2 = three ? L.gate[1] : L.cout, act2 = three ? L.gate[2] : L.act;
    FM_CHECK_ARG(!to.f32 && L.hid == 32 && stem2_supported(L.hid, cout2) && L.in_coff[0] == 0 && L.out_coff + L.cout <= to.c);
    FM_CHECK_ARG(!three || stem3_supported(cout2, L.cout));
    const char* w2 = net->weights + L.w2_off;
    const char* b2 = net->weights + L.b2_off;
    return launch_stem2(src, (const f16*)net->bufs[L.in[0]], ti.c, (f16*)net->bufs[L.out], to.c, L.out_coff,
                        (const f16*)(net->weights + L.w_off), (const float*)(net->weights + L.b_off), (const f16*)w2,
                        (const float*)b2, batch, ti.h, ti.w, to.h / 1, to.w / 1, cout2, L.gate[0], act2, s, three ? L.cout : 0,
                        three ? (const f16*)(w2 + (size_t)cout2 * 288 * 2) : nullptr,
                        three ? (const float*)(b2 + (size_t)cout2 * 4) : nullptr, L.act);
}

int launch_stempool_layer(const fm_layer& L, const StemSrc& src, const NetState* net, int batch, hipStream_t s) {
    const fm_tensor& ti = net->tensors[L.in[0]];
    const fm_tensor& to = net->tensors[L.out];
    FM_CHECK_ARG(!ti.f32 && !to.f32 && L.k == 7 && L.stride == 2 && L.pad == 3 && L.act == FM_ACT_RELU && L.in_coff[0] == 0 &&
                 (L.gate[0] == 0 || L.gate[0] == 1) && stempool_supported(L.cout, L.gate[0]) && L.out_coff + ((L.cout + 7) & ~7) <= to.c);
    FM_CHECK_ARG(L.b_off >= 0 && (size_t)L.w_off + (size_t)((L.cout + 31) & ~31) * 208 * 2 <= net->weight_bytes &&
                 (size_t)L.b_off + (size_t)((L.cout + 31) & ~31) * 4 <= net->weight_bytes);
    const int hc = (ti.h + 6 - 7) / 2 + 1, wc = (ti.w + 6 - 7) / 2 + 1;
    return launch_stempool_src(src, (const f16*)net->bufs[L.in[0]], ti.c, 0, (f16*)net->bufs[L.out], to.c, L.out_coff,
                               (const f16*)(net->weights + L.w_off), (const float*)(net->weights + L.b_off), batch, ti.h, ti.w,
                               hc, wc, to.h, to.w, L.gate[0], L.cout, s);
}

int fm_net_run_stem_from(fm_ctx* ctx, NetState* net, const StemSrc& src, int batch) {
    FM_CHECK_ARG(ctx && net && !net->layers.empty() && batch >= 1 && batch <= net->max_batch);
    const fm_layer& L = net->layers[0];
    FM_CHECK_ARG(L.op == FM_OP_STEMCONV || L.op == FM_OP_STEM2 || L.op == FM_OP_STEMPOOL);
    const fm_tensor& ti = net->tensors[L.in[0]];
    const fm_tensor& to = net->tensors[L.out];
    if (L.op == FM_OP_STEM2) {
        FM_CHECK_ARG(src.kind != 2);
        return launch_stem2_layer(L, src, net, batch, net->stream);
    }
    if (L.op == FM_OP_STEMPOOL) {
        FM_CHECK_ARG(src.kind == 2);
        return launch_stempool_layer(L, src, net, batch, net->stream);
    }
    return launch_stemconv_src(src, (const f16*)net->bufs[L.in[0]], ti.c, 0, (f16*)net->bufs[L.out], to.c, L.out_coff,
                               (const f16*)(net->weights + L.w_off), (const float*)(net->weights + L.b_off), batch, ti.h,
                               ti.w, to.h, to.w, L.k, L.stride, L.pad, L.cout, L.act, net->stream);
}

extern "C" int fm_net_run(fm_ctx* ctx, int which, int batch) {
    FM_CHECK_ARG(ctx && (which >= 0 && which < FM_NET_EXTRACTOR_B + FM_MAX_EXTRA_EXTRACTORS));
    NetState* net = net_slot(ctx, which);
    FM_CHECK_ARG(net != nullptr && batch >= 0 && batch <= net->max_batch);
    if (batch == 0) return 0;
    if (!net->use_graphs || !ctx->opt_use_graphs) return run_layers_eager(ctx, net, batch);
    const NetState::GraphKey key{((long)batch << 32) | (unsigned)net->emb_offset, net->first, net->last, net->set};
    for (auto& g : net->graphs)
        if (g.first == key) {
            FM_HIP(hipGraphLaunch(g.second, net->stream));
            return 0;
        }
    int rc = run_layers_eager(ctx, net, batch);
    if (rc) return rc;
    FM_HIP(hipStreamSynchronize(net->stream));
    hipGraph_t graph = nullptr;
    hipGraphExec_t exec = nullptr;
    if (hipStreamBeginCapture(net->stream, hipStreamCaptureModeThreadLocal) != hipSuccess) {
        (void)hipGetLastError();
        net->use_graphs = false;
        return 0;
    }
    rc = run_layers_eager(ctx, net, batch);
    const hipError_t ec = hipStreamEndCapture(net->stream, &graph);
    if (rc != 0 || ec != hipSuccess || graph == nullptr ||
        hipGraphInstantiate(&exec, graph, nullptr, nullptr, 0) != hipSuccess) {
        (void)hipGetLastError();
        if (graph) (void)hipGraphDestroy(graph);
        net->use_graphs = false;
        return rc;
    }
    (void)hipGraphDestroy(graph);
    net->graphs.emplace_back(key, exec);
    return 0;
}

extern "C" int fm_net_tensor_write(fm_ctx* ctx, int which, int tensor, const void* host, size_t bytes) {
    FM_CHECK_ARG(ctx && (which >= 0 && which < FM_NET_EXTRACTOR_B + FM_MAX_EXTRA_EXTRACTORS) && host);
    NetState* net = net_slot(ctx, which);
    FM_CHECK_ARG(net && tensor >= 0 && tensor < (int)net->tensors.size());
    const fm_tensor& t = net->tensors[tensor];
    FM_CHECK_ARG(bytes <= (size_t)net->max_batch * t.h * t.w * t.c * elem_size(t));
    int rc = fm_net_sync(net);
    if (rc) return rc;
    FM_HIP(hipMemcpy(net->bufs[tensor], host, bytes, hipMemcpyHostToDevice));
    if (!net->bufs_b.empty() && net->bufs_b[tensor] != net->bufs[tensor])
        FM_HIP(hipMemcpy(net->bufs_b[tensor], host, bytes, hipMemcpyHostToDevice));
    return 0;
}

extern "C" int fm_net_tensor_read(fm_ctx* ctx, int which, int tensor, void* host, size_t bytes) {
    FM_CHECK_ARG(ctx && (which >= 0 && which < FM_NET_EXTRACTOR_B + FM_MAX_EXTRA_EXTRACTORS) && host);
    NetState* net = net_slot(ctx, which);
    FM_CHECK_ARG(net && tensor >= 0 && tensor < (int)net->tensors.size());
    const fm_tensor& t = net->tensors[tensor];
    FM_CHECK_ARG(bytes <= (size_t)net->max_batch * t.h * t.w * t.c * elem_size(t));
    int rc = fm_net_sync(net);
    if (rc) return rc;
    FM_HIP(hipMemcpy(host, net->bufs[tensor], bytes, hipMemcpyDeviceToHost));
    return 0;
}

extern "C" int fm_net_read_embeddings(fm_ctx* ctx, int n, float* host) {
    FM_CHECK_ARG(ctx && n >= 0 && n <= ctx->emb_cap);
    if (n == 0) return 0;
    FM_CHECK_ARG(host);
    FM_HIP(hipStreamSynchronize(ctx->s_ext));
    FM_HIP(hipMemcpy(host, ctx->emb, sizeof(float) * (size_t)n * ctx->feat_dim, hipMemcpyDeviceToHost));
    ctx->emb_n = n;
    return 0;
}

extern "C" int fm_net_read_embeddings_mirror(fm_ctx* ctx, int n, float* host) {
    FM_CHECK_ARG(ctx && n >= 0 && n <= ctx->emb_cap);
    if (n == 0) return 0;
    FM_CHECK_ARG(host && ctx->emb_host);
    FM_HIP(hipStreamSynchronize(ctx->s_ext));
    memcpy(host, ctx->emb_host, sizeof(float) * (size_t)n * ctx->feat_dim);
    return 0;
}

static void layer_cost(const NetState* net, const fm_layer& L, int B, double* flops, double* bytes) {
    const fm_tensor& ti = net->tensors[L.in[0]];
    const fm_tensor& to = net->tensors[L.out];
    const double pin = (double)B * ti.h * ti.w, pout = (double)B * to.h * to.w;
    *flops = 0;
    *bytes = 0;
    switch (L.op) {
        case FM_OP_CONV:
        case FM_OP_CONVS:
// ... 181 lines not shown
```

### fastmot_amd/csrc/ostail.hip

```cpp
#include "net.h"
#include <atomic>

namespace {

typedef float f32x16 __attribute__((ext_vector_type(16)));

#ifdef FM_OST_TIMING
__device__ long long g_ost_stamps[48];
#define OST_STAMP(i) if (blockIdx.x == 0 && threadIdx.x == 0) g_ost_stamps[i] = wall_clock64();
#else
#define OST_STAMP(i)
#endif

constexpr int MH = 16, MW = 8, HW = MH * MW;
constexpr int CI = 96, MID = 32, CO = 128, FD = 512;
constexpr int TS = CO + 8;
constexpr int S = MID + 8;
constexpr int RW = MW + 2, YPOS = (MH + 2) * RW;
constexpr int FRAG = 512;

constexpr int H_W1A = 0;
constexpr int H_PWA = H_W1A + 6 * FRAG;
constexpr int H_DWA = H_PWA + 20 * FRAG;
constexpr int H_W3A = H_DWA + 10 * 9 * MID;
constexpr int H_W1B = H_W3A + 32 * FRAG;
constexpr int H_PWB = H_W1B + 8 * FRAG;
constexpr int H_DWB = H_PWB + 20 * FRAG;
constexpr int H_W3B = H_DWB + 10 * 9 * MID;
constexpr int H_W5 = H_W3B + 8 * FRAG;
constexpr int H_FC = H_W5 + 32 * FRAG;
constexpr int H_TOTAL = H_FC + FD * CO;
constexpr int GATE_F = 2 * MID + 4 + 2 * MID + MID;
constexpr int F_B1A = 0, F_BCA = F_B1A + MID, F_GA = F_BCA + 10 * MID, F_B3A = F_GA + GATE_F, F_B1B = F_B3A + CO,
              F_BCB = F_B1B + MID, F_GB = F_BCB + 10 * MID, F_B3B = F_GB + GATE_F, F_B5 = F_B3B + CO, F_FC = F_B5 + CO,
              F_TOTAL = F_FC + FD;

constexpr int L_R1 = 0, L_EX = L_R1 + HW * TS, L_R2 = L_R1 + 4 * YPOS * S, L_ZB = L_R2 + HW * TS, L_DW = L_ZB + 4 * HW * S,
              L_HALFS = L_DW + 10 * 9 * MID;
constexpr int LF_BC = 0, LF_GP = LF_BC + 10 * MID, LF_GAP = LF_GP + GATE_F, LF_HID = LF_GAP + 4 * MID, LF_GATE = LF_HID + 8, LF_HGAP = LF_GATE + 4 * MID,
              LF_FEAT = LF_HGAP + CO, LF_RED = LF_FEAT + FD, LF_PART = LF_RED + 16, L_FLOATS = LF_PART + 4 * 32 * MID;
constexpr size_t LDS_BYTES = (size_t)L_HALFS * 2 + (size_t)L_FLOATS * 4;
static_assert(HW * TS * 2 >= 64 * CO * 4, "the head's partial sums live in R2");
static_assert(L_HALFS % 8 == 0 && LDS_BYTES <= 160 * 1024, "LDS budget");

template <int KS>
__device__ __forceinline__ void load_frags(f16x8 (&a)[KS], const f16* __restrict__ wf, int lane) {
#pragma unroll
    for (int ks = 0; ks < KS; ++ks) a[ks] = *reinterpret_cast<const f16x8*>(wf + ks * FRAG + lane * 8);
}
template <int KS>
__device__ __forceinline__ f32x16 mm_tile(const f16x8 (&a)[KS], const f16* xrow) {
    f32x16 acc;
#pragma unroll
    for (int r = 0; r < 16; ++r) acc[r] = 0.f;
#pragma unroll
    for (int ks = 0; ks < KS; ++ks)
        acc = __builtin_amdgcn_mfma_f32_32x32x16_f16(a[ks], *reinterpret_cast<const f16x8*>(xrow + ks * 16), acc, 0, 0, 0);
    return acc;
}

__device__ __forceinline__ void load_bias(float4 (&b)[4], const float* __restrict__ bias, int fh) {
#pragma unroll
    for (int g = 0; g < 4; ++g) b[g] = *reinterpret_cast<const float4*>(bias + g * 8 + fh * 4);
}

template <bool BIAS, bool RES, bool RELU>
__device__ __forceinline__ void store_tile(const f32x16& acc, const float4 (&bias)[4], f16* drow, int fh) {
#pragma unroll
    for (int g = 0; g < 4; ++g) {
        const int c0 = g * 8 + fh * 4;
        float v[4];
#pragma unroll
        for (int e = 0; e < 4; ++e) v[e] = acc[g * 4 + e];
        if constexpr (BIAS) {
            v[0] += bias[g].x; v[1] += bias[g].y; v[2] += bias[g].z; v[3] += bias[g].w;
        }
        union { f16 h[4]; uint2 u; } pk;
        if constexpr (RES) {
            pk.u = *reinterpret_cast<const uint2*>(drow + c0);
#pragma unroll
            for (int e = 0; e < 4; ++e) v[e] += (float)pk.h[e];
        }
#pragma unroll
        for (int e = 0; e < 4; ++e) pk.h[e] = (f16)(RELU ? fmaxf(v[e], 0.f) : v[e]);
        *reinterpret_cast<uint2*>(drow + c0) = pk.u;
    }
}

template <int CTRL>
__device__ __forceinline__ float dpp_add(float t) {
    return t + __int_as_float(__builtin_amdgcn_update_dpp(0, __float_as_int(t), CTRL, 0xf, 0xf, true));
}
template <int N>
__device__ __forceinline__ float lanes_sum(float t) {
    t = dpp_add<0xB1>(t);
    t = dpp_add<0x4E>(t);
    if constexpr (N >= 8) t = dpp_add<0x141>(t);
    if constexpr (N >= 16) t = dpp_add<0x140>(t);
    return t;
}

__device__ __forceinline__ void lds_barrier() {
    asm volatile("s_waitcnt lgkmcnt(0)\n\ts_barrier" ::: "memory");
}

__device__ __forceinline__ void zero_halfs(f16* p, int n8, int tid) {
    for (int i = tid; i < n8; i += 1024) reinterpret_cast<uint4*>(p)[i] = make_uint4(0u, 0u, 0u, 0u);
}

template <int PXW>
__device__ __forceinline__ void dw_items(const f16* ys, f16* zb, const f16* dwl, const float* bcl, float* part, int lvl, int nact,
                                         int tid) {
    constexpr int IPS = HW / PXW * 8;
    if (tid < nact * IPS) {
        const int s = lvl + tid / IPS, r = tid % IPS, ch0 = (r & 7) * 4, strip = r >> 3;
        const int y = strip / (MW / PXW), x0 = (strip % (MW / PXW)) * PXW;
        const int pset = s * (s + 1) / 2 + lvl;
        const f16* yp = ys + (s * YPOS + y * RW + x0) * S + ch0;
        uint2 raw[3][PXW + 2], kh[9];
#pragma unroll
        for (int dy = 0; dy < 3; ++dy)
#pragma unroll
            for (int dx = 0; dx < PXW + 2; ++dx) raw[dy][dx] = *reinterpret_cast<const uint2*>(yp + (dy * RW + dx) * S);
#pragma unroll
        for (int t = 0; t < 9; ++t) kh[t] = *reinterpret_cast<const uint2*>(dwl + (pset * 9 + t) * MID + ch0);
        const float4 bias = *reinterpret_cast<const float4*>(bcl + pset * MID + ch0);
        float gs[4] = {0.f, 0.f, 0.f, 0.f};
#pragma unroll
        for (int p = 0; p < PXW; ++p) {
            float acc[4] = {bias.x, bias.y, bias.z, bias.w};
#pragma unroll
            for (int dy = 0; dy < 3; ++dy)
#pragma unroll
                for (int dx = 0; dx < 3; ++dx)
                    fma_mix_nh<4>(reinterpret_cast<const uint32_t*>(&raw[dy][p + dx]),
                                  reinterpret_cast<const uint32_t*>(&kh[dy * 3 + dx]), acc);
            union { f16 h[4]; uint2 u; } pk;
#pragma unroll
            for (int e = 0; e < 4; ++e) pk.h[e] = (f16)fmaxf(acc[e], 0.f);
            *reinterpret_cast<uint2*>(zb + (s * HW + y * MW + x0 + p) * S + ch0) = pk.u;
            if (lvl == s) {
#pragma unroll
                for (int e = 0; e < 4; ++e) gs[e] += (float)pk.h[e];
            }
        }
        if (lvl == s) {
            if constexpr (PXW == 2) {
#pragma unroll
                for (int e = 0; e < 4; ++e) {
                    const float o = __shfl_xor(gs[e], 8);
                    gs[e] = (strip & 1) ? o + gs[e] : gs[e] + o;
                }
            }
            if (PXW == 4 || !(strip & 1))
                *reinterpret_cast<float4*>(part + (s * 32 + strip * PXW / 4) * MID + ch0) = make_float4(gs[0], gs[1], gs[2], gs[3]);
        }
    }
}

__device__ __forceinline__ void os_chain(const f16* __restrict__ pw, f16x8 (&a0)[2], const f16* dwl, const float* bcl, f16* ys,
                                         f16* zb, float* part, int tid, int stamp0) {
    const int lane = tid & 63, wave = tid >> 6, frow = lane & 31, fh = lane >> 5;
    (void)stamp0;
    const float4 nob[4] = {};
    f16x8 an[2];
    for (int lvl = 0; lvl < 4; ++lvl) {
        const int nact = 4 - lvl;
        if (wave < nact * 4) {
            const int s = lvl + (wave >> 2), mt = wave & 3, px = mt * 32 + frow;
            const f16* xrow = zb + ((lvl == 0 ? 0 : s * HW) + px) * S + fh * 8;
            const f32x16 acc = mm_tile<2>(a0, xrow);
            store_tile<false, false, false>(acc, nob, ys + (s * YPOS + ((px >> 3) + 1) * RW + (px & 7) + 1) * S, fh);
        }
        lds_barrier();
        OST_STAMP(stamp0 + 2 * lvl)
        if (wave < (nact - 1) * 4) {
            const int s = lvl + 1 + (wave >> 2);
            load_frags<2>(an, pw + (s * (s + 1) / 2 + lvl + 1) * 2 * FRAG, lane);
        }
        dw_items<4>(ys, zb, dwl, bcl, part, lvl, nact, tid);
        a0[0] = an[0];
        a0[1] = an[1];
        lds_barrier();
        OST_STAMP(stamp0 + 2 * lvl + 1)
    }
}

// ... 266 lines not shown
```

### fastmot_amd/csrc/pixel_source.h

```cpp
#pragma once
#include "net.h"

#define FM_FRAME_SLACK 16
typedef uint64_t fm_u64_unaligned __attribute__((aligned(1)));
__device__ __forceinline__ uint64_t load_px2(const uint8_t* p) { return *reinterpret_cast<const fm_u64_unaligned*>(p); }

__device__ __forceinline__ void det_input_pixel(const uint8_t* __restrict__ frame, int fw, int fh, int x, int y,
                                                int roi_x, int roi_y, int roi_w, int roi_h, float rgb[3]) {
    const int rx0 = x - roi_x, ry0 = y - roi_y;
    const bool in_roi = !(rx0 < 0 || ry0 < 0 || rx0 >= roi_w || ry0 >= roi_h);
    const int rx = min(max(rx0, 0), roi_w - 1), ry = min(max(ry0, 0), roi_h - 1);
    const double zy = (double)fh / roi_h, zx = (double)fw / roi_w;
    const double sy = ry * zy + (zy - 1.) / 2., sx = rx * zx + (zx - 1.) / 2.;
    const double fy = floor(sy), fx = floor(sx);
    const double wy = sy - fy, wx = sx - fx;
    int y0 = (int)fy, x0 = (int)fx, y1 = y0 + 1, x1 = x0 + 1;
    y0 = min(max(y0, 0), fh - 1); y1 = min(max(y1, 0), fh - 1);
    x0 = min(max(x0, 0), fw - 1); x1 = min(max(x1, 0), fw - 1);
    const uint64_t q0 = load_px2(frame + ((size_t)y0 * fw + x0) * 3), q1 = load_px2(frame + ((size_t)y1 * fw + x0) * 3);
    const int sh = x1 == x0 ? 0 : 24;
#pragma unroll
    for (int c = 0; c < 3; ++c) {
        const int p00 = (int)((q0 >> (8 * c)) & 255), p01 = (int)((q0 >> (sh + 8 * c)) & 255);
        const int p10 = (int)((q1 >> (8 * c)) & 255), p11 = (int)((q1 >> (sh + 8 * c)) & 255);
// ... 20 lines not shown
    return c;
}

__device__ __forceinline__ bool crop_u8_pixel(const uint8_t* __restrict__ frame, int fw, int fh,
                                              const double* __restrict__ bx, int x, int y, int ow, int oh, int bgr[3]) {
    int x1 = max((int)bx[0], 0), y1 = max((int)bx[1], 0);
    int x2 = max((int)bx[2], 0), y2 = max((int)bx[3], 0);
    x2 = min(x2 + 1, fw); y2 = min(y2 + 1, fh);
    const int cw = x2 - x1, ch = y2 - y1;
    if (!(cw > 0 && ch > 0)) return false;
    const ResizeCoef cx = lin_coef(x, (double)cw / ow, cw);
    const ResizeCoef cy = lin_coef(y, (double)ch / oh, ch);
    const int sx1 = min(cx.s + 1, cw - 1), sy1 = min(cy.s + 1, ch - 1);
    const bool area2 = cw == 2 * ow && ch == 2 * oh;
    const int ax = area2 ? 2 * x : cx.s, ay0 = area2 ? 2 * y : cy.s, ay1 = area2 ? 2 * y + 1 : sy1;
    const uint64_t q0 = load_px2(frame + ((size_t)(y1 + ay0) * fw + x1 + ax) * 3);
    const uint64_t q1 = load_px2(frame + ((size_t)(y1 + ay1) * fw + x1 + ax) * 3);
    const int sh = (area2 || sx1 != cx.s) ? 24 : 0;
#pragma unroll
    for (int c = 0; c < 3; ++c) {
        const int a0 = (int)((q0 >> (8 * c)) & 255), a1 = (int)((q0 >> (sh + 8 * c)) & 255);
        const int b0 = (int)((q1 >> (8 * c)) & 255), b1 = (int)((q1 >> (sh + 8 * c)) & 255);
        if (area2) {
            bgr[c] = (a0 + a1 + b0 + b1 + 2) >> 2;
        } else {
            const int S0 = a0 * cx.a0 + a1 * cx.a1;
            const int S1 = b0 * cx.a0 + b1 * cx.a1;
            const int v = (((cy.a0 * (S0 >> 4)) >> 16) + ((cy.a1 * (S1 >> 4)) >> 16) + 2) >> 2;
            bgr[c] = min(max(v, 0), 255);
        }
    }
    return true;
}

__device__ __forceinline__ f16 crop_normalise(int u8, int rc) {
    const double mean[3] = {0.485, 0.456, 0.406}, stdv[3] = {0.229, 0.224, 0.225};
    return (f16)(float)(((double)u8 / 255. - mean[rc]) / stdv[rc]);
}

__device__ __forceinline__ void crop_input_pixel(const uint8_t* __restrict__ frame, int fw, int fh,
                                                 const double* __restrict__ bx, int x, int y, int ow, int oh, f16x8& o) {
#pragma unroll
    for (int e = 0; e < 8; ++e) o[e] = (f16)0.f;
    int bgr[3];
    if (crop_u8_pixel(frame, fw, fh, bx, x, y, ow, oh, bgr)) {
#pragma unroll
        for (int c = 0; c < 3; ++c) o[2 - c] = crop_normalise(bgr[c], 2 - c);
    }
}

struct StemSrc {
    int kind;
    const uint8_t* frame[FM_MAX_DET_BATCH];
    int fw, fh;
    int roi_x[FM_MAX_DET_BATCH], roi_y[FM_MAX_DET_BATCH];
    int roi_w, roi_h;
    const double* boxes;
    int32_t* zero4[FM_MAX_DET_BATCH];
};

template <typename T>
__device__ __forceinline__ T pick_sample(const T (&a)[FM_MAX_DET_BATCH], int i) {
    T r = a[0];
#pragma unroll
    for (int k = 1; k < FM_MAX_DET_BATCH; ++k) r = i == k ? a[k] : r;
    return r;
}

int launch_stemconv_src(const StemSrc& src, const f16* in, int in_cs, int in_coff, f16* out, int out_cs, int out_coff,
                        const f16* w, const float* bias, int N, int H, int W, int Ho, int Wo, int k, int stride, int pad,
                        int cout, int act, hipStream_t s);
int launch_stem2(const StemSrc& src, const f16* in, int in_cs, f16* out, int out_cs, int out_coff, const f16* w1,
                 const float* b1, const f16* w2, const float* b2, int N, int H, int W, int Ho, int Wo, int cout, int act1,
                 int act2, hipStream_t s, int cout3 = 0, const f16* w3 = nullptr, const float* b3 = nullptr, int act3 = 0);
bool stem2_supported(int mid, int cout);
bool stem3_supported(int cout2, int cout3);
int launch_stem2_layer(const fm_layer& L, const StemSrc& src, const NetState* net, int batch, hipStream_t s);
bool stempool_supported(int cout, int ppad);
int launch_stempool_src(const StemSrc& src, const f16* in, int in_cs, int in_coff, f16* out, int out_cs, int out_coff,
                        const f16* w, const float* bias, int N, int H, int W, int Hc, int Wc, int Hp, int Wp, int ppad,
                        int cout, hipStream_t s);
int launch_stempool_layer(const fm_layer& L, const StemSrc& src, const NetState* net, int batch, hipStream_t s);
bool fm_net_stem_fusable(const NetState* net, int input_tensor);
int fm_net_run_stem_from(fm_ctx* ctx, NetState* net, const StemSrc& src, int batch);
```

### include/fastmot_hip.h

```cpp
#ifndef FASTMOT_HIP_H
#define FASTMOT_HIP_H

#include <stddef.h>
#include <stdint.h>

#ifdef __cplusplus
extern "C" {
#endif

typedef struct fm_ctx fm_ctx;

int fm_ctx_create(int device, fm_ctx** out);
int fm_ctx_destroy(fm_ctx* ctx);
const char* fm_last_error(void);
int fm_device_count(void);
int fm_device_pci_bus_id(int device, char* buf, int buflen);
int fm_ctx_synchronize(fm_ctx* ctx);
int fm_ctx_bind_thread(fm_ctx* ctx);
int fm_ctx_set_option(fm_ctx* ctx, const char* key, int value);
int fm_ctx_get_option(fm_ctx* ctx, const char* key, int* value);
int fm_net_front_info(fm_ctx* ctx, int* k, long long* bytes, long long* passes);
int fm_trace_start(fm_ctx* ctx, int cap, int64_t* host_ns);
int fm_trace_read(fm_ctx* ctx, int cap, int32_t* tags, float* ms, int* n);
int fm_device_info(fm_ctx* ctx, char* buf, int buflen);
// ... 88 lines not shown
int fm_stage_cost_host(int stage, int nT, int nD, const double* feat, const double* maha, const double* iou,
                       const uint8_t* row_has_feat, const int64_t* det_label, const uint8_t* det_occluded,
                       int nr, const int32_t* rows, int nc, const int32_t* cols, const int64_t* row_labels,
                       double motion_weight, double max_cost, double fill_val, double* cost);
int fm_unmatched_order(int n, const int32_t* matched, int n_matched, int32_t* out);

int fm_lap(fm_ctx* ctx, const double* cost, int nr, int nc,
           int32_t* m_rows, int32_t* m_cols, int* n_match);
int fm_greedy(fm_ctx* ctx, const double* cost, int nr, int nc, double max_cost,
              int32_t* m_rows, int32_t* m_cols, int* n_match);
int fm_iou_dist(fm_ctx* ctx, int na, const double* a, int nb, const double* b, double* out);

enum { FM_NET_DETECTOR = 0, FM_NET_EXTRACTOR = 1,
       FM_NET_EXTRACTOR_B = 2  };
#define FM_MAX_EXTRA_EXTRACTORS 3
enum {
    FM_OP_CONV = 0,
    FM_OP_DWCONV3 = 1,
    FM_OP_MAXPOOL = 2,
    FM_OP_AVGPOOL = 3,
    FM_OP_UPSAMPLE2 = 4,
    FM_OP_COPY = 5,
    FM_OP_GATE = 6,
    FM_OP_GATE_SUM = 7,
    FM_OP_HEAD = 8,
    FM_OP_SPP = 10,
    FM_OP_LITECONV = 9,
    FM_OP_STEMCONV = 12,
    FM_OP_ADD = 13,
    FM_OP_RESBLOCK = 14,
    FM_OP_CONVS = 15,
    FM_OP_LITECHAIN = 16,
    FM_OP_CONVD = 17,
    FM_OP_STEM2 = 18,
    FM_OP_PAIR11 = 19,
    FM_OP_OSTAIL = 20,
    FM_OP_DWCONV = 21,
    FM_OP_SEPCONV = 22,
    FM_OP_POOLHEAD = 23,
    FM_OP_STEMPOOL = 24,
    FM_OP_INSTNORM = 25,
    FM_OP_CONVIN = 26,
    FM_OP_NONLOCAL = 27,
    FM_OP_GATED_SUM = 11
};
enum { FM_ACT_LINEAR = 0, FM_ACT_LEAKY = 1, FM_ACT_MISH = 2, FM_ACT_RELU = 3, FM_ACT_LOGISTIC = 4,
       FM_ACT_SWISH = 5, FM_ACT_RELU6 = 6  };
enum { FM_RES_NONE = 0, FM_RES_AFTER_ACT = 1, FM_RES_BEFORE_ACT = 2,
       FM_RES_BEFORE_NORM = 3  };

typedef struct fm_tensor {
    int32_t h, w, c;
    int32_t f32;
    int64_t offset;
} fm_tensor;

typedef struct fm_layer {
    int32_t op;
    int32_t n_in;
    int32_t in[4], in_coff[4];
    int32_t out, out_coff;
    int32_t res, res_coff, res_mode;
    int32_t cin, cout, k, stride, pad, act;
    int32_t hid;
    int32_t up;
    int32_t gate[4];
    int64_t w_off, b_off, w2_off, b2_off;
} fm_layer;

int fm_net_create(fm_ctx* ctx, int which, int max_batch, int n_tensors, const fm_tensor* tensors,
                  int n_layers, const fm_layer* layers, const void* weights, size_t weight_bytes,
                  int n_gates, int gate_channels, size_t arena_bytes);
int fm_net_destroy(fm_ctx* ctx, int which);
int fm_net_run(fm_ctx* ctx, int which, int batch);
int fm_net_tensor_write(fm_ctx* ctx, int which, int tensor, const void* host, size_t bytes);
int fm_net_tensor_read(fm_ctx* ctx, int which, int tensor, void* host, size_t bytes);
int fm_net_read_embeddings(fm_ctx* ctx, int n, float* host);
int fm_net_read_embeddings_mirror(fm_ctx* ctx, int n, float* host);
int fm_net_cost(fm_ctx* ctx, int which, int batch, double* flops, double* bytes);
int fm_net_profile(fm_ctx* ctx, int which, int batch, int iters, double* conv_ms, double* other_ms,
                   int* n_conv, int* n_other);

int fm_net_profile_layers(fm_ctx* ctx, int which, int batch, int iters, double* out);

int fm_frame_configure(fm_ctx* ctx, int width, int height, int ring_size);
int fm_frame_upload(fm_ctx* ctx, const uint8_t* bgr);
int fm_host_alloc(size_t bytes, void** out);
int fm_host_free(void* p);
int fm_frame_upload_next(fm_ctx* ctx, const uint8_t* bgr);
int fm_frame_ring_select_next(fm_ctx* ctx, int index);
int fm_frame_promote_next(fm_ctx* ctx);
int fm_detect_async_next(fm_ctx* ctx);
#define FM_MAX_DET_BATCH 4
int fm_frame_upload_ahead(fm_ctx* ctx, int k, const uint8_t* bgr);
int fm_frame_ring_select_ahead(fm_ctx* ctx, int k, int index);
int fm_detect_async_ahead(fm_ctx* ctx, int n);
int fm_frame_ring_store(fm_ctx* ctx, int index, const uint8_t* bgr);
int fm_frame_ring_select(fm_ctx* ctx, int index);
int fm_frame_read(fm_ctx* ctx, uint8_t* bgr);
#define FM_NV12_BT601 0
#define FM_NV12_BT709 1
int fm_frame_upload_nv12(fm_ctx* ctx, const uint8_t* y, const uint8_t* uv, int pitch, int matrix);
int fm_frame_upload_ahead_nv12(fm_ctx* ctx, int k, const uint8_t* y, const uint8_t* uv, int pitch, int matrix);
int fm_frame_ring_store_nv12(fm_ctx* ctx, int index, const uint8_t* y, const uint8_t* uv, int pitch, int matrix);

#define FM_ERR_UNSUPPORTED (-4)
#define FM_JPEG_UNSUPPORTED_PROGRESSIVE 1
#define FM_JPEG_UNSUPPORTED_ARITHMETIC 2
#define FM_JPEG_UNSUPPORTED_PROCESS 3
#define FM_JPEG_UNSUPPORTED_PRECISION 4
#define FM_JPEG_UNSUPPORTED_COMPONENTS 5
#define FM_JPEG_UNSUPPORTED_COLORSPACE 6
#define FM_JPEG_UNSUPPORTED_SAMPLING 7
#define FM_JPEG_UNSUPPORTED_SCANS 8
struct fm_jpeg_info {
    int32_t width, height;
    int32_t ncomp;
    int32_t hsamp[3], vsamp[3];
    int32_t mcu_w, mcu_h;
    int32_t mcus_x, mcus_y;
    int32_t restart_interval;
    int32_t blocks_w[3], blocks_h[3];
    int32_t unsupported;
    int64_t coef_offset[3];
    int64_t coef_count;
};
int fm_jpeg_info(const uint8_t* data, size_t n, struct fm_jpeg_info* out);
int fm_jpeg_entropy_decode(const uint8_t* data, size_t n, const struct fm_jpeg_info* info, int16_t* coef, uint16_t* qt);
int fm_frame_upload_jpeg(fm_ctx* ctx, const struct fm_jpeg_info* info, const int16_t* coef, const uint16_t* qt);
int fm_frame_upload_ahead_jpeg(fm_ctx* ctx, int k, const struct fm_jpeg_info* info, const int16_t* coef, const uint16_t* qt);
int fm_frame_ring_store_jpeg(fm_ctx* ctx, int index, const struct fm_jpeg_info* info, const int16_t* coef, const uint16_t* qt);

#define FM_SRC_BGR 0
#define FM_SRC_NV12 1
#define FM_SRC_JPEG 2
#define FM_SRC_MAX_DIM 16384
struct fm_frame_src {
    int32_t kind, width, height;
    const uint8_t* bgr;
    const uint8_t *y, *uv;
    int32_t pitch, matrix;
    const struct fm_jpeg_info* info;
    const int16_t* coef;
    const uint16_t* qt;
};
int fm_frame_upload_src(fm_ctx* ctx, const struct fm_frame_src* src);
int fm_frame_upload_ahead_src(fm_ctx* ctx, int k, const struct fm_frame_src* src);
int fm_frame_ring_store_src(fm_ctx* ctx, int index, const struct fm_frame_src* src);

#define FM_YUV_420 0
#define FM_YUV_422 1
#define FM_YUV_444 2
#define FM_YUV_MONO 3
struct fm_frame_planar {
    int32_t width, height, chroma, matrix;
    const uint8_t *y, *u, *v;
    int32_t pitch_y, pitch_c;
};
int fm_frame_upload_planar(fm_ctx* ctx, const struct fm_frame_planar* f);
int fm_frame_upload_ahead_planar(fm_ctx* ctx, int k, const struct fm_frame_planar* f);
int fm_frame_ring_store_planar(fm_ctx* ctx, int index, const struct fm_frame_planar* f);

#define FM_PACKED_RGB 0
#define FM_PACKED_BGR 1
#define FM_PACKED_RGBX 2
#define FM_PACKED_BGRX 3
// ... 303 lines not shown
```

Baseline: 1078.

## Add planner fusing runs of pointwise convs and avgpool into one LDS kernel

Adds a network planner that finds chains of up to three 1x1 convolutions, optionally with a 2x2 avgpool between them, and runs each chain in a single MFMA kernel. The intermediate activations stay in LDS, and an intermediate is only written to global memory when a later layer reads it. Arena tensors whose bytes alias are moved to their own allocations when fusion requires it. The aim is to save kernel launches and global round trips for intermediates, at the cost of more LDS use and lower occupancy. The feature sits behind opt_net_fuse_runs, which defaults to 0.

New measurement: 1064. 1.2% lower.

```diff
diff --git a/fastmot_amd/_lib.py b/fastmot_amd/_lib.py
--- a/fastmot_amd/_lib.py
+++ b/fastmot_amd/_lib.py
@@ -233,6 +233,11 @@
         k, b, n = C.c_int(0), C.c_longlong(0), C.c_longlong(0)
         check(self.lib.fm_net_front_info(self._ctx, C.byref(k), C.byref(b), C.byref(n)))
         return k.value, b.value, n.value
+
+    def net_plan_info(self, which):
+        n, d = C.c_int(0), C.c_int(0)
+        check(self.lib.fm_net_plan_info(self._ctx, C.c_int(which), C.byref(n), C.byref(d)))
+        return n.value, d.value
 
     def trace_start(self, cap=20000):
         t0 = C.c_int64(0)
diff --git a/fastmot_amd/build.py b/fastmot_amd/build.py
--- a/fastmot_amd/build.py
+++ b/fastmot_amd/build.py
@@ -11,7 +11,8 @@
          '-Wno-unused-result'] + os.environ.get('FASTMOT_EXTRA_HIPCC_FLAGS', '').split()
 
 
-FILE_FLAGS = {'flow.hip': ['-fno-slp-vectorize'], 'diag.hip': ['-fno-slp-vectorize'], 'reidhead_gem.hip': ['-fno-slp-vectorize']}
+FILE_FLAGS = {'flow.hip': ['-fno-slp-vectorize'], 'diag.hip': ['-fno-slp-vectorize'], 'reidhead_gem.hip': ['-fno-slp-vectorize'],
+              'pwrun.hip': ['-fno-slp-vectorize']}
 
 
 def sources():
diff --git a/fastmot_amd/csrc/common.h b/fastmot_amd/csrc/common.h
--- a/fastmot_amd/csrc/common.h
+++ b/fastmot_amd/csrc/common.h
@@ -94,6 +94,7 @@
     int opt_host_lap_elems = 262144;
     int opt_use_graphs = 1;
     int opt_fused_input = 1;
+    int opt_net_fuse_runs = 0;
     int opt_net_timing = 0;
     int opt_nms_general = 0;
     int opt_det_front_ahead = 1;
diff --git a/fastmot_amd/csrc/convd.hip b/fastmot_amd/csrc/convd.hip
--- a/fastmot_amd/csrc/convd.hip
+++ b/fastmot_amd/csrc/convd.hip
@@ -301,16 +301,7 @@
             const int row = orow + ps * ROWS;
             const int pix = p0 + row;
             if (row >= BN || pix >= p.P) continue;
-#pragma unroll
-            for (int e = 0; e < 8; ++e) {
-                v[ps][e] += bias8[e];
-                if (p.res_mode == RES_BEFORE_ACT) v[ps][e] += r[ps][e];
-            }
-            apply_act_n<8>(v[ps], p.act);
-            if (p.res_mode == RES_AFTER_ACT) {
-#pragma unroll
-                for (int e = 0; e < 8; ++e) v[ps][e] += r[ps][e];
-            }
+            conv_epilogue_n<8>(v[ps], bias8, r[ps], p.act, p.res_mode);
             if (p.out32) {
                 float* dst = p.out32 + (size_t)pix * p.out_cs + p.out_coff + co;
                 *reinterpret_cast<float4*>(dst) = make_float4(v[ps][0], v[ps][1], v[ps][2], v[ps][3]);
diff --git a/fastmot_amd/csrc/ctx.hip b/fastmot_amd/csrc/ctx.hip
--- a/fastmot_amd/csrc/ctx.hip
+++ b/fastmot_amd/csrc/ctx.hip
@@ -28,6 +28,10 @@
     }
     else if (!strcmp(key, "fused_input")) ctx->opt_fused_input = value != 0;
     else if (!strcmp(key, "net_timing")) ctx->opt_net_timing = value;
+    else if (!strcmp(key, "net_fuse_runs")) {
+        FM_CHECK_ARG(value <= 2);
+        ctx->opt_net_fuse_runs = value;
+    }
     else if (!strcmp(key, "det_front_ahead") || !strcmp(key, "det_front_stream")) {
         FM_CHECK_ARG(value <= (key[10] == 'a' ? 2 : 1));
         (key[10] == 'a' ? ctx->opt_det_front_ahead : ctx->opt_det_front_stream) = value;
@@ -136,6 +140,7 @@
     if (const char* e = getenv("FASTMOT_HOST_LAP")) ctx->opt_host_lap_elems = atoi(e);
     if (const char* e = getenv("FASTMOT_GRAPHS")) ctx->opt_use_graphs = atoi(e);
     if (const char* e = getenv("FASTMOT_FUSED_INPUT")) ctx->opt_fused_input = atoi(e) != 0;
+    if (const char* e = getenv("FASTMOT_NET_FUSE_RUNS")) ctx->opt_net_fuse_runs = std::min(std::max(atoi(e), 0), 2);
     if (const char* e = getenv("FASTMOT_FRONT_AHEAD")) ctx->opt_det_front_ahead = std::min(std::max(atoi(e), 0), 2);
     if (const char* e = getenv("FASTMOT_FRONT_STREAM")) ctx->opt_det_front_stream = atoi(e) == 1;
     int prio_lo = 0, prio_hi = 0;
diff --git a/fastmot_amd/csrc/detect.hip b/fastmot_amd/csrc/detect.hip
--- a/fastmot_amd/csrc/detect.hip
+++ b/fastmot_amd/csrc/detect.hip
@@ -712,10 +712,11 @@
         fm_net_select(net, se, set);
         if (timing) FM_HIP(hipEventRecord(d->evf0[d->wr], se));
         fm_trace_mark(ctx, se, 11);
-        if ((rc = fm_net_run_stem_from(ctx, net, src, n))) return rc;
+        int used = 0;
+        if ((rc = fm_net_run_stem_from(ctx, net, src, n, &used))) return rc;
         fm_trace_mark(ctx, se, 15);
         if (K > 1) {
-            net->first = 1;
+            net->first = used;
             net->last = K;
             if ((rc = fm_net_run_internal(ctx, FM_NET_DETECTOR, n))) return rc;
         }
@@ -743,9 +744,10 @@
         if (fused) {
             if (timing) FM_HIP(hipEventRecord(d->ev0[d->wr], s));
             fm_trace_mark(ctx, s, 11);
-            if ((rc = fm_net_run_stem_from(ctx, net, src, n))) return rc;
+            int used = 0;
+            if ((rc = fm_net_run_stem_from(ctx, net, src, n, &used))) return rc;
             fm_trace_mark(ctx, s, 15);
-            net->first = 1;
+            net->first = used;
             rc = fm_net_run_internal(ctx, FM_NET_DETECTOR, n);
             net->first = 0;
             if (rc) return rc;
diff --git a/fastmot_amd/csrc/extract.hip b/fastmot_amd/csrc/extract.hip
--- a/fastmot_amd/csrc/extract.hip
+++ b/fastmot_amd/csrc/extract.hip
@@ -86,9 +86,10 @@
         StemSrc src{};
         src.kind = 2; src.frame[0] = ctx->frame_cur; src.fw = ctx->frame_w; src.fh = ctx->frame_h;
         src.boxes = e->boxes_host + (size_t)off * 4;
-        int rc = fm_net_run_stem_from(ctx, ni, src, b);
-        if (rc) return rc;
-        ni->first = 1;
+        int used = 0;
+        int rc = fm_net_run_stem_from(ctx, ni, src, b, &used);
+        if (rc) return rc;
+        ni->first = used;
         return 0;
     }
     hipLaunchKernelGGL(crop_resize_kernel, dim3((e->in_w + 127) / 128, e->in_h, b), dim3(128), 0, si,
diff --git a/fastmot_amd/csrc/net.h b/fastmot_amd/csrc/net.h
--- a/fastmot_amd/csrc/net.h
+++ b/fastmot_amd/csrc/net.h
@@ -30,6 +30,11 @@
 
 int launch_conv(const ConvParams& p, float* ws, size_t ws_floats, hipStream_t s);
 
+enum { RUN_SINGLE = 0, RUN_POINTWISE = 1, RUN_STEMPOOL = 2 };
+struct NetRun {
+    int first, n, kind;
+};
+
 struct NetState {
     int which = 0, max_batch = 0;
     std::vector<fm_tensor> tensors;
@@ -45,8 +50,8 @@
     size_t ws_floats = 0;
     struct GraphKey {
         long batch_emb;
-        int first, last, set;
-        bool operator==(const GraphKey& o) const { return batch_emb == o.batch_emb && first == o.first && last == o.last && set == o.set; }
+        int first, last, set, fuse;
+        bool operator==(const GraphKey& o) const { return batch_emb == o.batch_emb && first == o.first && last == o.last && set == o.set && fuse == o.fuse; }
     };
     std::vector<std::pair<GraphKey, hipGraphExec_t>> graphs;
     bool use_graphs = true;
@@ -65,7 +70,33 @@
     hipStream_t home = nullptr;
     hipStream_t front_stream = nullptr;
     long front_passes = 0;
-};
+    std::vector<NetRun> runs;
+    std::vector<char> stored;
+    std::vector<char> moved;
+    bool own_alloc(size_t t) const { return tensors[t].offset < 0 || (t < moved.size() && moved[t]); }
+};
+
+void fm_net_plan(int which, int max_batch, const std::vector<fm_tensor>& tensors, const std::vector<fm_layer>& layers,
+                 std::vector<NetRun>* runs, std::vector<char>* stored, std::vector<char>* moved);
+
+constexpr int PWRUN_MAX = 3;
+struct PwStage {
+    const f16* w;
+    const float* bias;
+    f16* out;       int out_cs, out_coff;
+    const f16* res; int res_cs, res_coff, res_mode;
+    int K, cout, act;
+    int pool;
+    f16* pout;      int pout_cs, pout_coff;
+};
+struct PwRunParams {
+    const f16* in;  int in_cs, in_coff;
+    int H, W, n_stage;
+    int lds_a, lds_b, lds_w;
+    PwStage st[PWRUN_MAX];
+};
+bool pwrun_supported(int n, const int* K, const int* cout, const int* pool, int H, int W);
+int launch_pwrun(const PwRunParams& p, int N, hipStream_t s);
 
 int fm_net_front_prepare(fm_ctx* ctx, NetState* net, int request, int* k);
 void fm_net_select(NetState* net, hipStream_t s, int set);
@@ -190,3 +221,21 @@
         default: break;
     }
 }
+
+template <int N>
+__device__ __forceinline__ void conv_epilogue_n(float* v, const float* bias, const float* r, int act, int res_mode) {
+#pragma unroll
+    for (int e = 0; e < N; ++e) {
+        v[e] += bias[e];
+        if (res_mode == RES_BEFORE_ACT) v[e] += r[e];
+    }
+    apply_act_n<N>(v, act);
+    if (res_mode == RES_AFTER_ACT) {
+#pragma unroll
+        for (int e = 0; e < N; ++e) v[e] += r[e];
+    }
+}
+
+__device__ __forceinline__ void lds_barrier() {
+    asm volatile("s_waitcnt lgkmcnt(0)\n\ts_barrier" ::: "memory");
+}
diff --git a/fastmot_amd/csrc/net.hip b/fastmot_amd/csrc/net.hip
--- a/fastmot_amd/csrc/net.hip
+++ b/fastmot_amd/csrc/net.hip
@@ -72,7 +72,7 @@
 void fm_net_free(NetState* n) {
     if (!n) return;
     for (size_t i = 0; i < n->bufs.size(); ++i)
-        if (n->bufs[i] && n->tensors[i].offset < 0 && !(i < n->in_front.size() && n->in_front[i])) (void)hipFree(n->bufs[i]);
+        if (n->bufs[i] && n->own_alloc(i) && !(i < n->in_front.size() && n->in_front[i])) (void)hipFree(n->bufs[i]);
     for (void* p : n->front_owned) (void)hipFree(p);
     if (n->arena) (void)hipFree(n->arena);
     if (n->weights) (void)hipFree(n->weights);
@@ -186,7 +186,7 @@
             net->front_owned.push_back(p);
             FM_HIP(hipMemset(p, 0, b));
         }
-        if (T.offset < 0) FM_HIP(hipFree(net->bufs[t]));
+        if (net->own_alloc(t)) FM_HIP(hipFree(net->bufs[t]));
         net->bufs[t] = two[0];
         net->bufs_b[t] = two[1];
         net->in_front[t] = 1;
@@ -229,11 +229,17 @@
         FM_HIP(hipMalloc(&net->arena, arena_bytes));
         FM_HIP(hipMemset(net->arena, 0, arena_bytes));
     }
+    for (const fm_tensor& t : net->tensors) FM_CHECK_ARG(t.h > 0 && t.w > 0 && t.c > 0 && t.c % 8 == 0);
+    for (const fm_layer& L : net->layers) {
+        FM_CHECK_ARG(L.out >= 0 && L.out < n_tensors && L.n_in >= 1 && L.n_in <= 4);
+        for (int i = 0; i < L.n_in; ++i) FM_CHECK_ARG(L.in[i] >= 0 && L.in[i] < n_tensors);
+        FM_CHECK_ARG(L.res_mode == FM_RES_NONE || (L.res >= 0 && L.res < n_tensors));
+    }
+    fm_net_plan(which, max_batch, net->tensors, net->layers, &net->runs, &net->stored, &net->moved);
     for (const fm_tensor& t : net->tensors) {
-        FM_CHECK_ARG(t.h > 0 && t.w > 0 && t.c > 0 && t.c % 8 == 0);
         void* b = nullptr;
         const size_t bytes = (size_t)max_batch * t.h * t.w * t.c * elem_size(t);
-        if (t.offset >= 0) {
+        if (t.offset >= 0 && !net->moved[&t - net->tensors.data()]) {
             FM_CHECK_ARG(t.offset % 256 == 0 && (size_t)t.offset + bytes <= arena_bytes);
             b = net->arena + t.offset;
         } else {
@@ -256,6 +262,7 @@
     net->weight_bytes = weight_bytes;
     net->n_gates = n_gates;
     net->gate_c = gate_channels;
+
     net->ws_floats = ((size_t)16 << 20) * (which == FM_NET_DETECTOR ? (size_t)std::min(max_batch, FM_MAX_DET_BATCH) : 1);
     FM_HIP(hipMalloc(&net->ws, net->ws_floats * sizeof(float)));
     if (n_gates > 0) {
@@ -573,16 +580,267 @@
     }
 }
 
+namespace {
+
+struct PlanView {
+    int t, coff, c;
+};
+bool chan_overlap(const PlanView& a, const PlanView& b) { return a.t == b.t && a.coff < b.coff + b.c && b.coff < a.coff + a.c; }
+
+struct Planner {
+    int max_batch;
+    const std::vector<fm_tensor>& T;
+    const std::vector<fm_layer>& Ls;
+
+    size_t bytes(int t) const { return (size_t)max_batch * T[t].h * T[t].w * T[t].c * (T[t].f32 ? 4 : 2); }
+    bool bytes_overlap(int t, int u) const {
+        if (t == u) return true;
+        if (T[t].offset < 0 || T[u].offset < 0) return false;
+        return (size_t)T[t].offset < (size_t)T[u].offset + bytes(u) && (size_t)T[u].offset < (size_t)T[t].offset + bytes(t);
+    }
+    bool shares_bytes(int t) const {
+        for (int u = 0; u < (int)T.size(); ++u)
+            if (u != t && bytes_overlap(t, u)) return true;
+        return false;
+    }
+    bool read_outside(const PlanView& v, int lo, int hi) const {
+        for (int j = 0; j < (int)Ls.size(); ++j) {
+            if (j >= lo && j < hi) continue;
+            const fm_layer& L = Ls[j];
+            for (int k = 0; k < L.n_in; ++k)
+                if (chan_overlap(v, PlanView{L.in[k], L.in_coff[k], std::max(L.cin, 1)})) return true;
+            if (L.res_mode != FM_RES_NONE && chan_overlap(v, PlanView{L.res, L.res_coff, std::max((L.cout + 7) & ~7, 1)})) return true;
+        }
+        return false;
+    }
+    PlanView out_view(const fm_layer& L) const { return PlanView{L.out, L.out_coff, L.op == FM_OP_AVGPOOL || L.op == FM_OP_MAXPOOL ? L.cin : (L.cout + 7) & ~7}; }
+    bool droppable(const fm_layer& L, int lo, int hi) const { return !read_outside(out_view(L), lo, hi) && shares_bytes(L.out); }
+
+    bool pointwise(const fm_layer& L) const {
+        if (L.op != FM_OP_CONVD || L.k != 1 || L.stride != 1 || L.pad != 0 || L.up > 1 || L.n_in != 1) return false;
+        const fm_tensor &ti = T[L.in[0]], &to = T[L.out];
+        if (ti.f32 || to.f32 || ti.h != to.h || ti.w != to.w || L.cin % 8 || L.in_coff[0] % 8 || L.out_coff % 8) return false;
+        if (L.in_coff[0] + L.cin > ti.c || L.out_coff + ((L.cout + 7) & ~7) > to.c) return false;
+        if (L.res_mode == FM_RES_NONE) return true;
+        if (L.res_mode != FM_RES_AFTER_ACT && L.res_mode != FM_RES_BEFORE_ACT) return false;
+        const fm_tensor& tr = T[L.res];
+        return !tr.f32 && tr.h == to.h && tr.w == to.w && L.res_coff % 8 == 0 && L.res_coff + ((L.cout + 7) & ~7) <= tr.c;
+    }
+
+    bool run_ok(int i, int len, std::vector<char>* stored, std::vector<char>* moved) const {
+        int K[PWRUN_MAX], cout[PWRUN_MAX], pool[PWRUN_MAX], n = 0, pending = 0;
+        std::vector<PlanView> reads, writes;
+        reads.push_back(PlanView{Ls[i].in[0], Ls[i].in_coff[0], Ls[i].cin});
+        for (int j = i; j < i + len; ++j) {
+            const fm_layer& L = Ls[j];
+            const bool st = j == i + len - 1 || !droppable(L, i, i + len);
+            (*stored)[j] = st;
+            if (st) writes.push_back(out_view(L));
+            if (L.op == FM_OP_AVGPOOL) { pending = 1; continue; }
+            if (n == PWRUN_MAX) return false;
+            K[n] = L.cin; cout[n] = L.cout; pool[n] = pending; pending = 0; ++n;
+            if (L.res_mode != FM_RES_NONE) reads.push_back(PlanView{L.res, L.res_coff, (L.cout + 7) & ~7});
+        }
+        if (n < 2 || pending || !pwrun_supported(n, K, cout, pool, T[Ls[i].in[0]].h, T[Ls[i].in[0]].w)) return false;
+        std::vector<int> mv;
+        for (size_t a = 0; a < writes.size(); ++a) {
+            for (const PlanView& r : reads) {
+                if (r.t == writes[a].t ? chan_overlap(r, writes[a]) : false) return false;
+                if (r.t != writes[a].t && bytes_overlap(r.t, writes[a].t)) mv.push_back(writes[a].t);
+            }
+            for (size_t b = a + 1; b < writes.size(); ++b) {
+                if (writes[b].t == writes[a].t ? chan_overlap(writes[b], writes[a]) : false) return false;
+                if (writes[b].t != writes[a].t && bytes_overlap(writes[b].t, writes[a].t)) mv.push_back(writes[b].t);
+            }
+        }
+        for (int t : mv) (*moved)[t] = 1;
+        return true;
+    }
+
+    int pointwise_run(int i, std::vector<char>* stored, std::vector<char>* moved) const {
+        const int nl = (int)Ls.size();
+        if (!pointwise(Ls[i])) return 1;
+        std::vector<int> ends;
+        std::vector<int> written{Ls[i].out};
+        PlanView prev = out_view(Ls[i]);
+        int h = T[Ls[i].out].h, w = T[Ls[i].out].w, j = i + 1, convs = 1;
+        bool pooled = false;
+        while (convs < PWRUN_MAX && j < nl) {
+            int jc = j;
+            PlanView src = prev;
+            const fm_layer& P = Ls[j];
+            const bool pool = !pooled && P.op == FM_OP_AVGPOOL && P.k == 2 && P.stride == 2 && P.pad == 0 && P.n_in == 1 && P.in[0] == prev.t &&
+                              P.in_coff[0] == prev.coff && P.cin == prev.c && h % 2 == 0 && w % 2 == 0 && !T[P.out].f32 &&
+                              T[P.out].h == h / 2 && T[P.out].w == w / 2 && P.out_coff % 8 == 0 && P.out_coff + P.cin <= T[P.out].c;
+            if (pool) {
+                src = out_view(P);
+                if (++jc >= nl) break;
+            }
+            const fm_layer& L = Ls[jc];
+            const int hh = pool ? h / 2 : h, ww = pool ? w / 2 : w;
+            if (!pointwise(L) || L.in[0] != src.t || L.in_coff[0] != src.coff || L.cin != src.c || T[L.in[0]].h != hh || T[L.in[0]].w != ww) break;
+            bool inner_res = false;
+            if (pool) written.push_back(P.out);
+            if (L.res_mode != FM_RES_NONE)
+                for (int t : written) inner_res |= t == L.res;
+            if (inner_res) break;
+            written.push_back(L.out);
+            pooled |= pool;
+            h = hh; w = ww;
+            prev = out_view(L);
+            j = jc + 1;
+            ++convs;
+            ends.push_back(j - i);
+        }
+        for (size_t e = ends.size(); e-- > 0;)
+            if (run_ok(i, ends[e], stored, moved)) return ends[e];
+        return 1;
+    }
+
+    bool stem_pool() const {
+        if (Ls.size() < 2) return false;
+        const fm_layer &S = Ls[0], &P = Ls[1];
+        const fm_tensor &ti = T[S.in[0]], &tc = T[S.out], &tp = T[P.out];
+        if (S.op != FM_OP_STEMCONV || S.k != 7 || S.stride != 2 || S.pad != 3 || S.act != FM_ACT_RELU || S.cout > 32 || S.n_in != 1 ||
+            S.in_coff[0] != 0 || ti.f32 || tc.f32 || tp.f32)
+            return false;
+        if (P.op != FM_OP_MAXPOOL || P.k != 3 || P.stride != 2 || (P.pad != 0 && P.pad != 1) || P.n_in != 1) return false;
+        const PlanView sv = out_view(S);
+        if (P.in[0] != sv.t || P.in_coff[0] != sv.coff || P.cin != sv.c || !stempool_supported(S.cout, P.pad)) return false;
+        const int hc = (ti.h + 6 - 7) / 2 + 1, wc = (ti.w + 6 - 7) / 2 + 1;
+        if (tc.h != hc || tc.w != wc || tp.h != (hc + P.pad + 1 - 3) / 2 + 1 || tp.w != (wc + P.pad + 1 - 3) / 2 + 1) return false;
+        if (P.out_coff % 8 || P.out_coff + sv.c > tp.c || P.out == S.in[0]) return false;
+        return droppable(S, 0, 2);
+    }
+};
+
+}
+
+void fm_net_plan(int which, int max_batch, const std::vector<fm_tensor>& tensors, const std::vector<fm_layer>& layers,
+                 std::vector<NetRun>* runs, std::vector<char>* stored, std::vector<char>* moved) {
+    const int nl = (int)layers.size();
+    runs->clear();
+    stored->assign(nl, 1);
+    moved->assign(tensors.size(), 0);
+    const Planner pl{max_batch, tensors, layers};
+    int i = 0;
+    if (which != FM_NET_DETECTOR && pl.stem_pool()) {
+        runs->push_back(NetRun{0, 2, RUN_STEMPOOL});
+        (*stored)[0] = 0;
+        i = 2;
+    }
+    while (i < nl) {
+        std::vector<char> st(nl, 1);
+        const int len = which != FM_NET_DETECTOR ? pl.pointwise_run(i, &st, moved) : 1;
+        if (len > 1)
+            for (int j = i; j < i + len; ++j) (*stored)[j] = st[j];
+        runs->push_back(NetRun{i, len, len > 1 ? RUN_POINTWISE : RUN_SINGLE});
+        i += len;
+    }
+}
+
+extern "C" int fm_net_plan_host(int which, int max_batch, int n_tensors, const fm_tensor* tensors, int n_layers, const fm_layer* layers,
+                                int* run_first, int* run_n, int* run_kind, int* stored, int* n_runs) {
+    FM_CHECK_ARG(which >= 0 && max_batch > 0 && n_tensors > 0 && n_layers > 0 && tensors && layers && run_first && run_n && run_kind &&
+                 stored && n_runs);
+    for (int i = 0; i < n_layers; ++i) {
+        const fm_layer& L = layers[i];
+        FM_CHECK_ARG(L.out >= 0 && L.out < n_tensors && L.n_in >= 1 && L.n_in <= 4);
+        for (int k = 0; k < L.n_in; ++k) FM_CHECK_ARG(L.in[k] >= 0 && L.in[k] < n_tensors);
+        FM_CHECK_ARG(L.res_mode == FM_RES_NONE || (L.res >= 0 && L.res < n_tensors));
+    }
+    std::vector<NetRun> runs;
+    std::vector<char> st, mv;
+    fm_net_plan(which, max_batch, std::vector<fm_tensor>(tensors, tensors + n_tensors), std::vector<fm_layer>(layers, layers + n_layers), &runs, &st, &mv);
+    for (size_t r = 0; r < runs.size(); ++r) {
+        run_first[r] = runs[r].first;
+        run_n[r] = runs[r].n;
+        run_kind[r] = runs[r].kind;
+    }
+    for (int i = 0; i < n_layers; ++i) stored[i] = st[i] ? (mv[layers[i].out] ? 2 : 1) : 0;
+    *n_runs = (int)runs.size();
+    return 0;
+}
+
+static bool fm_net_run_fused(const fm_ctx* ctx, const NetRun& r);
+extern "C" int fm_net_plan_info(fm_ctx* ctx, int which, int* launches, int* not_stored) {
+    FM_CHECK_ARG(ctx && (which >= 0 && which < FM_NET_EXTRACTOR_B + FM_MAX_EXTRA_EXTRACTORS) && launches && not_stored);
+    const NetState* net = net_slot(ctx, which);
+    FM_CHECK_ARG(net != nullptr);
+    *launches = *not_stored = 0;
+    for (const NetRun& r : net->runs) {
+        const bool fused = fm_net_run_fused(ctx, r);
+        *launches += fused ? 1 : r.n;
+        for (int j = r.first; fused && j < r.first + r.n; ++j) *not_stored += !net->stored[j];
+    }
+    return 0;
+}
+
+static int launch_pointwise_run(NetState* net, const NetRun& r, int B) {
+    PwRunParams p{};
+    const fm_layer& F = net->layers[r.first];
+    const fm_tensor& ti = net->tensors[F.in[0]];
+    p.in = (const f16*)net->bufs[F.in[0]]; p.in_cs = ti.c; p.in_coff = F.in_coff[0];
+    p.H = ti.h; p.W = ti.w;
+    const fm_layer* pool = nullptr;
+    for (int j = r.first; j < r.first + r.n; ++j) {
+        const fm_layer& L = net->layers[j];
+        if (L.op == FM_OP_AVGPOOL) { pool = &L; continue; }
+        FM_CHECK_ARG(p.n_stage < PWRUN_MAX && L.op == FM_OP_CONVD);
+        PwStage& st = p.st[p.n_stage++];
+        const size_t wbytes = (size_t)((L.cout + 31) / 32) * ((L.cin + 63) / 64) * 4096;
+        FM_CHECK_ARG(L.b_off >= 0 && (size_t)L.w_off + wbytes <= net->weight_bytes && (size_t)L.b_off + (size_t)((L.cout + 31) & ~31) * 4 <= net->weight_bytes);
+        st.w = (const f16*)(net->weights + L.w_off);
+        st.bias = (const float*)(net->weights + L.b_off);
+        if (net->stored[j]) { st.out = (f16*)net->bufs[L.out]; st.out_cs = net->tensors[L.out].c; st.out_coff = L.out_coff; }
+        st.res_mode = L.res_mode;
+        if (L.res_mode != FM_RES_NONE) { st.res = (const f16*)net->bufs[L.res]; st.res_cs = net->tensors[L.res].c; st.res_coff = L.res_coff; }
+        st.K = L.cin; st.cout = L.cout; st.act = L.act;
+        if (pool) {
+            st.pool = 1;
+            if (net->stored[pool - net->layers.data()]) { st.pout = (f16*)net->bufs[pool->out]; st.pout_cs = net->tensors[pool->out].c; st.pout_coff = pool->out_coff; }
+            pool = nullptr;
+        }
+    }
+    return launch_pwrun(p, B, net->stream);
+}
+
+static int launch_stem_run(NetState* net, const StemSrc& src, int B) {
+    const fm_layer &S = net->layers[0], &P = net->layers[1];
+    const fm_tensor &ti = net->tensors[S.in[0]], &tc = net->tensors[S.out], &tp = net->tensors[P.out];
+    FM_CHECK_ARG(S.b_off >= 0 && (size_t)S.w_off + (size_t)32 * 208 * 2 <= net->weight_bytes && (size_t)S.b_off + 32 * 4 <= net->weight_bytes);
+    return launch_stempool_src(src, (const f16*)net->bufs[S.in[0]], ti.c, 0, (f16*)net->bufs[P.out], tp.c, P.out_coff,
+                               (const f16*)(net->weights + S.w_off), (const float*)(net->weights + S.b_off), B, ti.h, ti.w, tc.h, tc.w,
+                               tp.h, tp.w, P.pad, S.cout, net->stream);
+}
+
 bool fm_net_writes_mirror(const NetState* net) {
     if (!net || net->layers.empty()) return false;
     const int op = net->layers.back().op;
     return op == FM_OP_HEAD || op == FM_OP_OSTAIL || op == FM_OP_POOLHEAD;
 }
 
+static bool fm_net_run_fused(const fm_ctx* ctx, const NetRun& r) {
+    return (r.kind == RUN_STEMPOOL && ctx->opt_net_fuse_runs >= 1) || (r.kind == RUN_POINTWISE && ctx->opt_net_fuse_runs >= 2);
+}
+
 static int run_layers_eager(fm_ctx* ctx, NetState* net, int batch) {
-    const size_t end = net->last > 0 ? (size_t)net->last : net->layers.size();
-    for (size_t i = (size_t)net->first; i < end; ++i) {
-        int rc = run_layer(ctx, net, net->layers[i], batch);
+    const int first = net->first, end = net->last > 0 ? net->last : (int)net->layers.size();
+    if (!ctx->opt_net_fuse_runs) {
+        for (int i = first; i < end; ++i) {
+            int rc = run_layer(ctx, net, net->layers[i], batch);
+            if (rc) return rc;
+        }
+        return 0;
+    }
+    for (const NetRun& r : net->runs) {
+        if (r.first + r.n <= first || r.first >= end) continue;
+        int rc = 0;
+        if (fm_net_run_fused(ctx, r) && r.first >= first && r.first + r.n <= end) {
+            rc = r.kind == RUN_POINTWISE ? launch_pointwise_run(net, r, batch) : launch_stem_run(net, StemSrc{}, batch);
+        } else {
+            for (int i = std::max(r.first, first); i < std::min(r.first + r.n, end) && !rc; ++i) rc = run_layer(ctx, net, net->layers[i], batch);
+        }
         if (rc) return rc;
     }
     return 0;
@@ -631,8 +889,14 @@
                                hc, wc, to.h, to.w, L.gate[0], L.cout, s);
 }
 
-int fm_net_run_stem_from(fm_ctx* ctx, NetState* net, const StemSrc& src, int batch) {
-    FM_CHECK_ARG(ctx && net && !net->layers.empty() && batch >= 1 && batch <= net->max_batch);
+int fm_net_run_stem_from(fm_ctx* ctx, NetState* net, const StemSrc& src, int batch, int* consumed) {
+    FM_CHECK_ARG(ctx && net && !net->layers.empty() && batch >= 1 && batch <= net->max_batch && consumed);
+    *consumed = 1;
+    if (ctx->opt_net_fuse_runs && !net->runs.empty() && net->runs[0].kind == RUN_STEMPOOL && (src.kind == 0 || src.kind == 2) &&
+        (net->last == 0 || net->last >= 2)) {
+        *consumed = 2;
+        return launch_stem_run(net, src, batch);
+    }
     const fm_layer& L = net->layers[0];
     FM_CHECK_ARG(L.op == FM_OP_STEMCONV || L.op == FM_OP_STEM2 || L.op == FM_OP_STEMPOOL);
     const fm_tensor& ti = net->tensors[L.in[0]];
@@ -656,7 +920,7 @@
     FM_CHECK_ARG(net != nullptr && batch >= 0 && batch <= net->max_batch);
     if (batch == 0) return 0;
     if (!net->use_graphs || !ctx->opt_use_graphs) return run_layers_eager(ctx, net, batch);
-    const NetState::GraphKey key{((long)batch << 32) | (unsigned)net->emb_offset, net->first, net->last, net->set};
+    const NetState::GraphKey key{((long)batch << 32) | (unsigned)net->emb_offset, net->first, net->last, net->set, ctx->opt_net_fuse_runs};
     for (auto& g : net->graphs)
         if (g.first == key) {
             FM_HIP(hipGraphLaunch(g.second, net->stream));
diff --git a/fastmot_amd/csrc/ostail.hip b/fastmot_amd/csrc/ostail.hip
--- a/fastmot_amd/csrc/ostail.hip
+++ b/fastmot_amd/csrc/ostail.hip
@@ -100,9 +100,6 @@
     return t;
 }
 
-__device__ __forceinline__ void lds_barrier() {
-    asm volatile("s_waitcnt lgkmcnt(0)\n\ts_barrier" ::: "memory");
-}
 
 __device__ __forceinline__ void zero_halfs(f16* p, int n8, int tid) {
     for (int i = tid; i < n8; i += 1024) reinterpret_cast<uint4*>(p)[i] = make_uint4(0u, 0u, 0u, 0u);
diff --git a/fastmot_amd/csrc/pixel_source.h b/fastmot_amd/csrc/pixel_source.h
--- a/fastmot_amd/csrc/pixel_source.h
+++ b/fastmot_amd/csrc/pixel_source.h
@@ -126,4 +126,4 @@
                         int cout, hipStream_t s);
 int launch_stempool_layer(const fm_layer& L, const StemSrc& src, const NetState* net, int batch, hipStream_t s);
 bool fm_net_stem_fusable(const NetState* net, int input_tensor);
-int fm_net_run_stem_from(fm_ctx* ctx, NetState* net, const StemSrc& src, int batch);
+int fm_net_run_stem_from(fm_ctx* ctx, NetState* net, const StemSrc& src, int batch, int* consumed);
diff --git a/fastmot_amd/csrc/pwrun.hip b/fastmot_amd/csrc/pwrun.hip
--- /dev/null
+++ b/fastmot_amd/csrc/pwrun.hip
@@ -0,0 +1,257 @@
+#include "net.h"
+#include <atomic>
+
+namespace {
+
+constexpr int PW_ROWS = 4;
+constexpr int PW_LDS_MAX = 160 * 1024;
+constexpr int PW_BIAS = 96;
+
+__host__ __device__ inline int pw_nk(int K) { return (K + 63) >> 6; }
+
+__device__ __forceinline__ unsigned pw_addr(int np32, int row, int chunk) {
+    return (unsigned)(chunk >> 3) * (unsigned)np32 * 4096u + (unsigned)row * 128u + (unsigned)(((chunk & 7) ^ ((row >> 1) & 7)) << 4);
+}
+
+typedef __attribute__((address_space(3))) void* lds_ptr;
+
+__global__ __launch_bounds__(256, 2) void pwrun_kernel(const PwRunParams p) {
+#if defined(__HIP_DEVICE_COMPILE__)
+    extern __shared__ __attribute__((aligned(16))) char smem[];
+    char* cur = smem;
+    char* nxt = smem + p.lds_a;
+    char* const wlds = smem + p.lds_a + p.lds_b;
+    float* const blds = reinterpret_cast<float*>(wlds + p.lds_w);
+    const int tid = threadIdx.x, lane = tid & 63;
+    const int w = __builtin_amdgcn_readfirstlane(tid >> 6);
+    const long n = blockIdx.y;
+    int H = p.H, W = p.W, y0 = blockIdx.x * PW_ROWS, trows = PW_ROWS;
+    int npix = min(trows, H - y0) * W;
+    int np32 = (trows * W + 31) >> 5;
+    long gpix = (n * H + y0) * (long)W;
+
+    constexpr unsigned OOB = 0x80000000u;
+    {
+        int woff = 0;
+        for (int s = 0; s < p.n_stage; ++s) {
+            const __amdgpu_buffer_rsrc_t rw = __builtin_amdgcn_make_buffer_rsrc(const_cast<f16*>(p.st[s].w), 0, 0x7fffffff, 0x00020000);
+            const int pieces = ((p.st[s].cout + 31) >> 5) * pw_nk(p.st[s].K) * 4;
+            for (int pc = w; pc < pieces; pc += 4)
+                __builtin_amdgcn_raw_ptr_buffer_load_lds(rw, (lds_ptr)(wlds + woff + pc * 1024), 16, (unsigned)pc * 1024u + (unsigned)lane * 16u, 0, 0, 0);
+            woff += pieces * 1024;
+            const int nb = ((p.st[s].cout + 31) >> 5) * 32;
+            if (tid < nb) blds[s * PW_BIAS + tid] = p.st[s].bias[tid];
+        }
+        const __amdgpu_buffer_rsrc_t ri = __builtin_amdgcn_make_buffer_rsrc(const_cast<f16*>(p.in), 0, 0x7fffffff, 0x00020000);
+        const int K = p.st[0].K, nk = pw_nk(K);
+        const int r8 = lane >> 3, slot = lane & 7;
+        for (int ks = 0; ks < nk; ++ks)
+            for (int pc = w; pc < np32 * 4; pc += 4) {
+                const int row = pc * 8 + r8, chunk = ks * 8 + (slot ^ ((row >> 1) & 7));
+                const unsigned vo = row < npix && chunk * 8 < K ? (unsigned)(((gpix + row) * p.in_cs + p.in_coff + chunk * 8) * 2) : OOB;
+                __builtin_amdgcn_raw_ptr_buffer_load_lds(ri, (lds_ptr)(cur + (ks * np32 * 4 + pc) * 1024), 16, vo, 0, 0, 0);
+            }
+    }
+
+    const int frow = lane & 31, fh = lane >> 5, swz = (lane >> 1) & 7;
+    unsigned koff[4];
+#pragma unroll
+    for (int j = 0; j < 4; ++j) koff[j] = (unsigned)(((2 * j + fh) ^ swz) << 4);
+    int woff = 0;
+
+#pragma unroll 1
+    for (int s = 0; s < p.n_stage; ++s) {
+        const PwStage& st = p.st[s];
+        const int K = st.K, nk = pw_nk(K);
+        const bool pooled = st.pool != 0;
+        const int Ws = pooled ? W >> 1 : W, trs = pooled ? trows >> 1 : trows, y0s = pooled ? y0 >> 1 : y0, Hs = pooled ? H >> 1 : H;
+        const int npixs = pooled ? (npix / W >> 1) * Ws : npix, np32s = (trs * Ws + 31) >> 5;
+        const long gpixs = (n * Hs + y0s) * (long)Ws;
+        const int ncb = (st.cout + 31) >> 5, cout_store = (st.cout + 7) & ~7;
+        const int pb = np32s >= 3 ? w : w % np32s;
+        const int cb0 = np32s >= 3 ? 0 : w / np32s, cstride = np32s >= 3 ? 1 : 4 / np32s;
+        const bool active = pb < np32s;
+        const int row = pb * 32 + frow;
+        const bool valid = row < npixs;
+        f16x4 rh[3][4];
+        if (st.res_mode != RES_NONE && active && valid) {
+#pragma unroll
+            for (int i = 0; i < 3; ++i) {
+                const int cb = cb0 + i * cstride;
+#pragma unroll
+                for (int q = 0; q < 4; ++q) {
+                    const int co = cb * 32 + 8 * q + 4 * fh;
+                    if (cb < ncb && co < cout_store) rh[i][q] = *reinterpret_cast<const f16x4*>(st.res + (gpixs + row) * st.res_cs + st.res_coff + co);
+                }
+            }
+        }
+        if (s == 0) {
+            asm volatile("s_waitcnt vmcnt(0)" ::: "memory");
+            __syncthreads();
+            asm volatile("" ::: "memory");
+        }
+        if (pooled) {
+            const int nch = nk * 8;
+            for (int i = tid; i < np32s * 32 * nch; i += 256) {
+                const int prow = i / nch, chunk = i - prow * nch;
+                uint4 o = make_uint4(0u, 0u, 0u, 0u);
+                if (prow < npixs && chunk * 8 < K) {
+                    const int py = prow / Ws, px = prow - py * Ws;
+                    float acc[8];
+#pragma unroll
+                    for (int e = 0; e < 8; ++e) acc[e] = 0.f;
+#pragma unroll
+                    for (int dy = 0; dy < 2; ++dy)
+#pragma unroll
+                        for (int dx = 0; dx < 2; ++dx) {
+                            float v[8];
+                            unpack8(*reinterpret_cast<const uint4*>(cur + pw_addr(np32, (2 * py + dy) * W + 2 * px + dx, chunk)), v);
+#pragma unroll
+                            for (int e = 0; e < 8; ++e) acc[e] = acc[e] + v[e];
+                        }
+                    const float inv = 1.f / 4.f;
+#pragma unroll
+                    for (int e = 0; e < 8; ++e) acc[e] *= inv;
+                    o = pack8(acc);
+                    if (st.pout) *reinterpret_cast<uint4*>(st.pout + (gpixs + prow) * st.pout_cs + st.pout_coff + chunk * 8) = o;
+                }
+                *reinterpret_cast<uint4*>(nxt + pw_addr(np32s, prow, chunk)) = o;
+            }
+            lds_barrier();
+            char* t = cur; cur = nxt; nxt = t;
+        }
+        H = Hs; W = Ws; y0 = y0s; trows = trs; npix = npixs; np32 = np32s; gpix = gpixs;
+
+        f32x16 acc[3];
+#pragma unroll
+        for (int i = 0; i < 3; ++i)
+#pragma unroll
+            for (int r = 0; r < 16; ++r) acc[i][r] = 0.f;
+        if (active) {
+            const char* bimg = cur + (unsigned)row * 128u;
+            const char* wimg = wlds + woff + frow * 128;
+            for (int ks = 0; ks < nk; ++ks) {
+#pragma unroll
+                for (int j = 0; j < 4; ++j) {
+                    const f16x8 bf = *reinterpret_cast<const f16x8*>(bimg + (unsigned)ks * (unsigned)np32 * 4096u + koff[j]);
+#pragma unroll
+                    for (int i = 0; i < 3; ++i) {
+                        const int cb = cb0 + i * cstride;
+                        if (cb < ncb) {
+                            const f16x8 af = *reinterpret_cast<const f16x8*>(wimg + (cb * nk + ks) * 4096 + koff[j]);
+                            acc[i] = __builtin_amdgcn_mfma_f32_32x32x16_f16(af, bf, acc[i], 0, 0, 0);
+                        }
+                    }
+                }
+            }
+        }
+        woff += ncb * nk * 4096;
+
+        {
+            const int c0 = cout_store >> 3, nz = pw_nk(cout_store) * 8 - c0;
+            for (int i = tid; i < np32 * 32 * nz; i += 256) {
+                const int zrow = i / nz, chunk = c0 + i - zrow * nz;
+                *reinterpret_cast<uint4*>(nxt + pw_addr(np32, zrow, chunk)) = make_uint4(0u, 0u, 0u, 0u);
+            }
+        }
+        if (active) {
+            const float* bias = blds + s * PW_BIAS;
+#pragma unroll
+            for (int i = 0; i < 3; ++i) {
+                const int cb = cb0 + i * cstride;
+                if (cb >= ncb) continue;
+#pragma unroll
+                for (int q = 0; q < 4; ++q) {
+                    const int co = cb * 32 + 8 * q + 4 * fh;
+                    if (co >= cout_store) continue;
+                    float v[4] = {acc[i][4 * q + 0], acc[i][4 * q + 1], acc[i][4 * q + 2], acc[i][4 * q + 3]};
+                    float b4[4], r4[4] = {0.f, 0.f, 0.f, 0.f};
+                    *reinterpret_cast<float4*>(b4) = *reinterpret_cast<const float4*>(bias + co);
+                    if (st.res_mode != RES_NONE && valid) {
+#pragma unroll
+                        for (int e = 0; e < 4; ++e) r4[e] = (float)rh[i][q][e];
+                    }
+                    conv_epilogue_n<4>(v, b4, r4, st.act, st.res_mode);
+                    f16x4 o;
+#pragma unroll
+                    for (int e = 0; e < 4; ++e) o[e] = (f16)v[e];
+                    *reinterpret_cast<f16x4*>(nxt + pw_addr(np32, row, co >> 3) + ((co >> 2) & 1) * 8) = o;
+                }
+            }
+        }
+        lds_barrier();
+        char* t = cur; cur = nxt; nxt = t;
+        if (st.out) {
+            const int nch = cout_store >> 3;
+            for (int i = tid; i < npix * nch; i += 256) {
+                const int orow = i / nch, chunk = i - orow * nch;
+                *reinterpret_cast<uint4*>(st.out + (gpix + orow) * st.out_cs + st.out_coff + chunk * 8) =
+                    *reinterpret_cast<const uint4*>(cur + pw_addr(np32, orow, chunk));
+            }
+        }
+    }
+#endif
+}
+
+bool pw_lds(int n, const int* K, const int* cout, const int* pool, int W, int* a, int* b, int* wb) {
+    int sz[2] = {0, 0}, which = 0, w = W, trows = PW_ROWS;
+    auto need = [&](int ch) {
+        const int bytes = ((trows * w + 31) >> 5) * 4096 * pw_nk(ch);
+        if (bytes > sz[which]) sz[which] = bytes;
+    };
+    need(K[0]);
+    for (int i = 0; i < n; ++i) {
+        if (pool[i]) {
+            w >>= 1; trows >>= 1; which ^= 1;
+            need(K[i]);
+        }
+        which ^= 1;
+        need((cout[i] + 7) & ~7);
+    }
+    *a = sz[0]; *b = sz[1]; *wb = 0;
+    for (int i = 0; i < n; ++i) *wb += ((cout[i] + 31) >> 5) * pw_nk(K[i]) * 4096;
+    return sz[0] + sz[1] + *wb + PWRUN_MAX * PW_BIAS * 4 <= PW_LDS_MAX;
+}
+
+}
+
+bool pwrun_supported(int n, const int* K, const int* cout, const int* pool, int H, int W) {
+    if (n < 1 || n > PWRUN_MAX || H < 1 || W < 1 || W > 32 || pool[0]) return false;
+    int pools = 0, h = H, w = W;
+    for (int i = 0; i < n; ++i) {
+        if (K[i] < 8 || K[i] % 8 || K[i] > 192 || cout[i] < 1 || cout[i] > 96) return false;
+        if (i && K[i] != ((cout[i - 1] + 7) & ~7)) return false;
+        if (pool[i]) {
+            if (++pools > 1 || h % 2 || w % 2) return false;
+            h /= 2; w /= 2;
+        }
+    }
+    int a, b, wb;
+    return pw_lds(n, K, cout, pool, W, &a, &b, &wb);
+}
+
+int launch_pwrun(const PwRunParams& p, int N, hipStream_t s) {
+    int K[PWRUN_MAX], cout[PWRUN_MAX], pool[PWRUN_MAX];
+    FM_CHECK_ARG(p.n_stage >= 1 && p.n_stage <= PWRUN_MAX && N >= 1 && N <= 65535 && p.in && p.in_cs % 8 == 0 && p.in_coff % 8 == 0);
+    for (int i = 0; i < p.n_stage; ++i) {
+        const PwStage& st = p.st[i];
+        K[i] = st.K; cout[i] = st.cout; pool[i] = st.pool;
+        FM_CHECK_ARG(st.w && st.bias && (!st.out || (st.out_cs % 8 == 0 && st.out_coff % 8 == 0)));
+        FM_CHECK_ARG(st.res_mode == RES_NONE || (st.res && st.res_cs % 8 == 0 && st.res_coff % 8 == 0));
+        FM_CHECK_ARG(!st.pout || (st.pool && st.pout_cs % 8 == 0 && st.pout_coff % 8 == 0));
+    }
+    FM_CHECK_ARG(pwrun_supported(p.n_stage, K, cout, pool, p.H, p.W) && (p.st[p.n_stage - 1].out != nullptr));
+    PwRunParams q = p;
+    pw_lds(p.n_stage, K, cout, pool, p.W, &q.lds_a, &q.lds_b, &q.lds_w);
+    FM_CHECK_ARG(((long)N * p.H * p.W * p.in_cs + p.in_coff) * 2 < (1L << 31));
+    static std::atomic<unsigned long long> configured{0};
+    int dev = 0;
+    FM_HIP(hipGetDevice(&dev));
+    if (dev >= 64 || !(configured.load(std::memory_order_relaxed) >> dev & 1)) {
+        FM_HIP(hipFuncSetAttribute(reinterpret_cast<const void*>(pwrun_kernel), hipFuncAttributeMaxDynamicSharedMemorySize, PW_LDS_MAX));
+        if (dev < 64) configured.fetch_or(1ull << dev, std::memory_order_relaxed);
+    }
+    hipLaunchKernelGGL(pwrun_kernel, dim3((p.H + PW_ROWS - 1) / PW_ROWS, N), dim3(256), (size_t)q.lds_a + q.lds_b + q.lds_w + PWRUN_MAX * PW_BIAS * 4, s, q);
+    FM_HIP(hipGetLastError());
+    return 0;
+}
diff --git a/include/fastmot_hip.h b/include/fastmot_hip.h
--- a/include/fastmot_hip.h
+++ b/include/fastmot_hip.h
@@ -194,6 +194,10 @@
                    int* n_conv, int* n_other);
 
 int fm_net_profile_layers(fm_ctx* ctx, int which, int batch, int iters, double* out);
+
+int fm_net_plan_info(fm_ctx* ctx, int which, int* launches, int* not_stored);
+int fm_net_plan_host(int which, int max_batch, int n_tensors, const fm_tensor* tensors, int n_layers, const fm_layer* layers,
+                     int* run_first, int* run_n, int* run_kind, int* stored, int* n_runs);
 
 int fm_frame_configure(fm_ctx* ctx, int width, int height, int ring_size);
 int fm_frame_upload(fm_ctx* ctx, const uint8_t* bgr);
```
